# HKUST-KnowComp/DualMessagePassing

Measured on AMD Instinct MI355X. Metric: (pattern,graph) pairs/sec DMPNN fwd+bwd hid=128, higher is better.
Workload: dtype f32

## Files before the change

dualmessagepassing_amd/_abi.py:

```python
import ctypes

c_int = ctypes.c_int
c_i32 = ctypes.c_int32
c_i64 = ctypes.c_int64
c_u64 = ctypes.c_uint64
c_f32 = ctypes.c_float
c_double = ctypes.c_double
c_ptr = ctypes.c_void_p
c_size = ctypes.c_size_t

ABI_VERSION = 97

DMP_COLLATE_MAX_JOBS = 4
DMP_POOL_MAX_JOBS = 4
DMP_REDUCE_MAX_SEGMENTS = 16
DMP_ADAMW_MAX_SKIP = 16
DMP_ADAMW_MAX_SEGMENTS = 1024
DMP_LOOKUP_MAX_JOBS = 8
DMP_CONCAT_MAX_JOBS = 12
DMP_GEMM_MAX_JOBS = 12
DMP_GEMM_MAX_TERMS = 3
DMP_ATB_MAX_JOBS = 8
DMP_MEM_MEAN, DMP_MEM_SUM, DMP_MEM_MAX = 0, 1, 2
DMP_LRP_MAX_NEIGHBOURS = 32
# ... 259 lines not shown
                                   c_ptr, c_ptr, c_int, c_ptr]),
    "dmp_adamw_step_segments": (c_int, [c_ptr, c_ptr, c_ptr, c_ptr, c_ptr, c_i64, c_ptr, c_ptr, c_int, c_ptr, c_ptr, c_ptr, c_double, c_double,
                                        c_double, c_double, c_ptr, c_int, c_ptr]),
    "dmp_adamw_step_guarded": (c_int, [c_ptr, c_ptr, c_ptr, c_ptr, c_ptr, c_i64, c_ptr, c_double, c_double, c_double, c_double,
                                       c_ptr, c_ptr, c_int, c_ptr, c_int, c_ptr]),
    "dmp_edge_select_build": (c_int, [c_ptr, c_ptr, c_ptr, c_ptr, c_i64, c_ptr, c_ptr, c_ptr, c_ptr]),
    "dmp_edge_select_nodes": (c_int, [c_ptr, c_ptr, c_ptr, c_ptr, c_i64, c_ptr, c_ptr, c_ptr, c_ptr]),
    "dmp_edge_fwd_fused": (c_int, [c_ptr, c_i64, c_ptr, c_i64, c_ptr, c_i64, c_i64, c_ptr, c_ptr, c_ptr, c_ptr,
                                   c_i64, c_int, c_f32, c_ptr, c_i64, c_ptr]),
    "dmp_edge_fwd_typed": (c_int, [c_ptr, c_i64, c_ptr, c_i64, c_ptr, c_i64, c_i64, c_ptr, c_ptr, c_ptr, c_ptr, c_ptr,
                                   c_ptr, c_i64, c_i64, c_int, c_f32, c_ptr, c_i64, c_ptr]),
    "dmp_bwd_z_typed_arow": (c_int, [c_ptr, c_i64, c_ptr, c_i64, c_ptr, c_i64, c_i64, c_ptr, c_i64, c_ptr, c_ptr, c_f32,
                                     c_f32, c_ptr, c_ptr, c_ptr, c_ptr, c_i64, c_i64, c_int, c_int, c_ptr, c_i64, c_ptr, c_i64, c_ptr]),
    "dmp_mask_slots": (c_int, [c_ptr, c_i64, c_ptr, c_i64, c_ptr, c_ptr]),
    "dmp_pool_relu_bwd_blocks": (c_i64, [c_i64, c_int]),
    "dmp_pool_relu_bwd": (c_int, [c_ptr, c_i64, c_ptr, c_i64, c_ptr, c_ptr, c_ptr, c_ptr, c_i64, c_i64, c_int, c_f32, c_ptr, c_i64,
                                  c_ptr, c_ptr, c_ptr]),
    "dmp_relu_bwd_gathered_colsum": (c_int, [c_ptr, c_i64, c_ptr, c_ptr, c_ptr, c_i64, c_i64, c_int, c_f32, c_ptr, c_i64, c_ptr, c_ptr]),
    "dmp_dev_set_exact_fp32": (None, [c_int]),
    "dmp_dev_get_exact_fp32": (c_int, []),
    "dmp_rel_gemm": (c_int, [c_ptr, c_i64, c_i64, c_ptr, c_i64, c_int, c_int, c_ptr, c_ptr, c_ptr, c_ptr, c_i64, c_ptr, c_i64,
                             c_int, c_ptr, c_i64, c_ptr]),
    "dmp_rel_atb_blocks": (c_i64, [c_int]),
    "dmp_rel_atb": (c_int, [c_ptr, c_i64, c_i64, c_ptr, c_i64, c_i64, c_ptr, c_ptr, c_ptr, c_ptr, c_int, c_i64, c_int, c_ptr, c_ptr]),
    "dmp_atb_typed_blocks_h": (c_i64, [c_i64, c_int]),
    "dmp_atb_rows_blocks_h": (c_i64, [c_i64, c_int, c_int, c_int]),
    "dmp_atb_rows_plain": (c_int, [c_ptr, c_i64, c_ptr, c_i64, c_ptr, c_i64, c_int, c_int, c_int, c_ptr, c_ptr]),
    "dmp_atb_rows_masked": (c_int, [c_ptr, c_i64, c_ptr, c_i64, c_ptr, c_ptr, c_i64, c_int, c_int, c_int, c_ptr, c_ptr, c_ptr]),
    "dmp_atb_jobs_blocks_h": (c_i64, [c_i64, c_int, c_int]),
    "dmp_atb_rows_jobs_h": (c_int, [_p(dmp_atb_job), c_int, c_i64, c_int, c_ptr, c_ptr, c_ptr, c_i64, c_ptr]),
    "dmp_atb_tile_jobs_blocks": (c_i64, [c_i64, c_int, c_int]),
    "dmp_mfma_partial_rows_h": (c_i64, [c_i64, c_int]),
    "dmp_gemm_k64": (c_int, [c_ptr, c_i64, c_ptr, c_i64, c_int, c_ptr, c_i64, c_i64, c_ptr]),
    "dmp_atb_typed": (c_int, [c_ptr, c_i64, c_ptr, c_i64, c_ptr, c_ptr, c_ptr, c_i64, c_i64, c_int, c_ptr, c_ptr, c_ptr]),
    "dmp_out_fwd_fused_rows": (c_int, [c_ptr, c_i64, c_ptr, c_i64, c_ptr, c_ptr, c_ptr, c_int, c_ptr, c_i64, c_i64, c_int, c_int, c_ptr,
                                       c_i64, c_ptr]),
    "dmp_bwd_h1_fused_rows": (c_int, [c_ptr, c_i64, c_ptr, c_i64, c_ptr, c_i64, c_ptr, c_ptr, c_ptr, c_int, c_i64, c_int, c_f32, c_ptr,
                                      c_i64, c_ptr, c_ptr, c_ptr]),
    "dmp_kept_rows_scratch_words": (c_i64, [c_i64]),
    "dmp_kept_rows": (c_int, [c_ptr, c_i64, c_int, c_ptr, c_ptr, c_ptr, c_ptr]),
    "dmp_l0_edge_fwd_rows": (c_int, [c_ptr, c_i64, c_int, c_ptr, c_i64, c_ptr, c_i64, c_ptr, c_ptr, c_ptr, c_ptr, c_ptr, c_ptr, c_i64, c_int,
                                     c_f32, c_ptr, c_i64, c_ptr]),
    "dmp_l0_bwd_w_rows": (c_int, [c_ptr, c_i64, c_int, c_ptr, c_ptr, c_i64, c_ptr, c_i64, c_ptr, c_ptr, c_i64, c_int, c_ptr, c_ptr]),
    "dmp_typed_partial_rows": (c_i64, [c_i64, c_int]),
    "dmp_out_fwd_typed": (c_int, [_p(dmp_typed_job), c_int, c_ptr, c_ptr, c_ptr, c_i64, c_i64, c_int, c_ptr]),
    "dmp_bwd_h1_typed": (c_int, [c_ptr, c_i64, c_ptr, c_i64, c_ptr, c_i64, c_ptr, c_ptr, c_ptr, c_i64, c_i64, c_int, c_f32, c_ptr, c_i64,
                                 c_ptr, c_ptr, c_ptr]),
    "dmp_kept_rows_jobs": (c_int, [_p(dmp_kept_job), c_int, c_ptr, c_ptr, c_ptr, c_ptr, c_i64, c_ptr, c_ptr, c_ptr, c_ptr]),
    "dmp_row_mask_bits_jobs": (c_int, [_p(dmp_rowmask_job), c_int, c_ptr]),
    "dmp_atb2_blocks": (c_i64, [c_i64, c_int]),
    "dmp_atb2_jobs": (c_int, [_p(dmp_atb2_job), c_int, c_ptr, c_ptr, c_ptr, c_i64, c_i64, c_int, c_ptr]),
    "dmp_bwd_z_w": (c_int, [c_ptr, c_i64, c_ptr, c_i64, c_ptr, c_i64, c_ptr, c_i64, c_i64, c_ptr, c_i64, c_ptr, c_ptr, c_f32, c_f32,
                            c_ptr, c_ptr, c_ptr, c_i64, c_i64, c_int, c_ptr, c_i64, c_ptr, c_i64, c_ptr, c_ptr]),
    "dmp_out_fwd_typed_codes": (c_int, [_p(dmp_typed_job), c_ptr, c_i64, c_int, c_ptr, c_i64, c_i64, c_i64, c_ptr, c_ptr, c_ptr, c_i64, c_i64, c_int, c_ptr]),
    "dmp_bwd_h1_w_blocks": (c_i64, [c_i64]),
    "dmp_bwd_h1_w": (c_int, [c_ptr, c_i64, c_ptr, c_i64, c_ptr, c_i64, c_ptr, c_ptr, c_i64, c_i64, c_int, c_f32, c_ptr, c_i64,
                             c_ptr, c_ptr, c_ptr, c_ptr]),
    "dmp_bwd_h1_w_max_codes": (c_int, []),
    "dmp_bwd_h1_w_codes": (c_int, [c_ptr, c_i64, c_ptr, c_i64, c_ptr, c_i64, c_ptr, c_ptr, c_i64, c_i64, c_int, c_f32, c_ptr, c_i64,
                                   c_ptr, c_ptr, c_ptr, c_ptr, c_i64, c_int, c_ptr, c_i64, c_i64, c_int, c_ptr, c_ptr]),
    "dmp_node_chain_blocks": (c_i64, [c_i64]),
    "dmp_node_chain_panel_words": (c_i64, []),
    "dmp_node_chain_pack": (c_int, [_p(dmp_chain_panel), c_int, c_ptr, c_ptr]),
    "dmp_node_chain_fwd": (c_int, [c_ptr, c_i64, c_ptr, c_i64, c_ptr, c_ptr, c_ptr, c_int, c_f32, c_ptr, c_ptr, c_i64, c_i64, c_int,
                                   c_ptr, c_i64, c_ptr, c_i64, c_ptr, c_i64, c_ptr]),
    "dmp_node_chain_bwd": (c_int, [c_ptr, c_i64, c_ptr, c_i64, c_ptr, c_i64, c_ptr, c_int, c_f32, c_ptr, c_ptr, c_i64, c_i64, c_int,
                                   c_ptr, c_i64, c_ptr, c_i64, c_ptr, c_i64, c_ptr, c_ptr, c_ptr]),
    "dmp_edge_mlp_fwd": (c_int, [c_ptr, c_i64, c_ptr, c_i64, c_ptr, c_i64, c_i64, c_ptr, c_ptr, c_ptr, c_ptr, c_i64, c_int, c_ptr, c_ptr, c_i64,
                                 c_ptr, c_ptr, c_ptr, c_i64, c_i64, c_int, c_f32, c_ptr, c_i64, c_ptr, c_i64, c_ptr]),
    "dmp_l0_edge_mlp_max_codes": (c_int, []),
    "dmp_l0_edge_mlp_fwd": (c_int, [c_ptr, c_i64, c_int, c_ptr, c_i64, c_int, c_i64, c_ptr, c_i64, c_i64, c_ptr, c_ptr, c_ptr, c_ptr, c_f32,
                                    c_ptr, c_i64, c_int, c_ptr, c_ptr, c_i64, c_i64, c_ptr, c_i64, c_i64, c_ptr, c_ptr, c_i64, c_i64, c_int,
                                    c_ptr, c_i64, c_ptr, c_i64, c_ptr]),
    "dmp_row_mask_bits": (c_int, [c_ptr, c_i64, c_ptr, c_ptr]),
    "dmp_row_mask_rows": (c_int, [c_ptr, c_i64, c_int, c_i64, c_ptr, c_ptr]),
    "dmp_bwd_z_fused": (c_int, [c_ptr, c_i64, c_ptr, c_i64, c_ptr, c_i64, c_i64, c_ptr, c_i64, c_ptr, c_ptr, c_ptr,
                                c_f32, c_f32, c_i64, c_int, c_ptr, c_i64, c_ptr]),
    "dmp_gemm_k128": (c_int, [c_ptr, c_i64, c_ptr, c_i64, c_int, c_ptr, c_i64, c_i64, c_int, c_ptr]),
    "dmp_edge_combine": (c_int, [c_ptr, c_i64, c_ptr, c_i64, c_ptr, c_ptr, c_ptr, c_ptr, c_ptr, c_i64,
                                 c_int, c_int, c_f32, c_ptr, c_i64, c_ptr]),
    "dmp_relu_bwd_g_colsum": (c_int, [c_ptr, c_i64, c_ptr, c_i64, c_ptr, c_ptr, c_i64, c_int, c_f32, c_ptr, c_i64,
                                      c_ptr, c_ptr]),
    "dmp_edge_combine_bwd_g": (c_int, [c_ptr, c_i64, c_ptr, c_ptr, c_i64, c_int, c_ptr, c_i64, c_ptr]),
    "dmp_compgcn_agg": (c_int, [c_ptr, c_i64, c_ptr, c_i64, c_ptr, c_ptr, c_ptr, c_ptr, c_i64, c_int, c_int,
                                c_ptr, c_i64, c_ptr]),
    "dmp_compgcn_agg_bwd": (c_int, [c_ptr, c_i64, c_ptr, c_i64, c_ptr, c_i64, c_ptr, c_ptr, c_ptr, c_ptr,
                                    c_i64, c_int, c_int, c_ptr, c_i64, c_ptr, c_i64, c_ptr]),
    "dmp_attn_supported_dh": (c_int, [c_int]),
    "dmp_attn_fwd": (c_int, [c_ptr, c_ptr, c_ptr, c_ptr, c_ptr, c_i64, c_i64, c_i64, c_int, c_int, c_f32, c_ptr, c_ptr, c_ptr, c_ptr]),
    "dmp_attn_bwd": (c_int, [c_ptr, c_ptr, c_ptr, c_ptr, c_ptr, c_ptr, c_ptr, c_ptr, c_i64, c_i64, c_i64, c_int, c_int, c_f32, c_ptr,
                             c_ptr, c_ptr, c_ptr, c_ptr]),
    "dmp_mem_init_fwd": (c_int, [c_ptr, c_i64, c_ptr, c_i64, c_ptr, c_i64, c_i64, c_int, c_int, c_int, c_int, c_int, c_ptr, c_ptr,
                                 c_ptr, c_ptr, c_ptr, c_ptr, c_ptr]),
    "dmp_mem_init_bwd": (c_int, [c_ptr, c_ptr, c_ptr, c_ptr, c_ptr, c_i64, c_i64, c_int, c_int, c_int, c_int, c_ptr, c_ptr, c_ptr]),
    "dmp_cnn_fwd": (c_int, [c_ptr, c_i64, c_i64, c_int, c_ptr, c_ptr, c_int, c_int, c_int, c_int, c_int, c_f32, c_ptr, c_int, c_ptr,
                            c_ptr, c_ptr, c_ptr, c_ptr]),
    "dmp_cnn_route_bwd": (c_int, [c_ptr, c_ptr, c_ptr, c_i64, c_i64, c_i64, c_int, c_int, c_int, c_f32, c_ptr, c_ptr]),
    "dmp_cnn_wgrad_chunks": (c_i64, [c_i64]),
    "dmp_cnn_wgrad": (c_int, [c_ptr, c_ptr, c_i64, c_i64, c_i64, c_int, c_int, c_int, c_ptr, c_ptr]),
    "dmp_rnn_fwd": (c_int, [c_ptr, c_ptr, c_ptr, c_ptr, c_ptr, c_i64, c_i64, c_int, c_int, c_int, c_ptr, c_ptr, c_ptr, c_ptr]),
    "dmp_rnn_bwd": (c_int, [c_ptr, c_ptr, c_ptr, c_ptr, c_ptr, c_i64, c_i64, c_int, c_int, c_int, c_ptr, c_ptr]),
    "dmp_relconv_supported": (c_int, [c_int, c_int]),
    "dmp_relconv_fwd": (c_int, [c_ptr, c_ptr, c_ptr, c_ptr, c_ptr, c_ptr, c_ptr, c_i64, c_int, c_int, c_int, c_int, c_int, c_ptr,
                                c_ptr]),
    "dmp_relconv_bwd": (c_int, [c_ptr, c_ptr, c_ptr, c_ptr, c_ptr, c_ptr, c_ptr, c_i64, c_int, c_int, c_int, c_int, c_int, c_ptr,
                                c_ptr]),
# ... 29 lines not shown
```

dualmessagepassing_amd/csrc/dmp_agg.hip:

```cpp
#include "dmp_common.h"

namespace dmp {

static thread_local char g_last_err[256] = "";
void set_last_hip_error(hipError_t e) {
  const char *s = hipGetErrorString(e);
  int i = 0;
  for (; s && s[i] && i < 255; ++i) g_last_err[i] = s[i];
  g_last_err[i] = 0;
}

namespace {

__device__ __forceinline__ float4 ld4(const float *p) {
  return *reinterpret_cast<const float4 *>(p);
}
__device__ __forceinline__ void st4(float *p, const float4 &v) {
  *reinterpret_cast<float4 *>(p) = v;
}
__device__ __forceinline__ float4 zero4() { return make_float4(0.f, 0.f, 0.f, 0.f); }
__device__ __forceinline__ void add4(float4 &a, const float4 &b) {
  a.x += b.x; a.y += b.y; a.z += b.z; a.w += b.w;
}
__device__ __forceinline__ float4 mul4(const float4 &a, float s) {
// ... 32 lines not shown
  if (rowlist) {
    if (row >= *rowcount) return;
    row = rowlist[row];
    if (!ptr_by_pos) prow = row;
  }
  const int beg = rowptr[prow], end = rowptr[prow + 1];
  for (int c0 = 0; c0 < H; c0 += G * 4) {
    const int c = c0 + lane * 4;
    const bool act = c < H;
    float4 a0 = zero4(), a1 = zero4();
    for (int base = beg; base < end; base += G) {
      const int cnt = min(G, end - base);
      int my = 0;
      float myw = 1.f;
      if (lane < cnt) {
        my = ent[base + lane];
        if (WEIGHTED) myw = ew[my >> 1];
      }
      for (int j = 0; j < cnt; j += U) {
        float4 v[U];
        int e[U];
#pragma unroll
        for (int k = 0; k < U; ++k) {
          e[k] = __shfl(my, min(j + k, G - 1), G);
          float w = 1.f;
          if (WEIGHTED) w = __shfl(myw, min(j + k, G - 1), G);
          if (act && j + k < cnt) {
            if (WEIGHTED && w == 0.f) {
              v[k] = zero4();
            } else {
              v[k] = ld4(M + (int64_t)(e[k] >> 1) * ldm + c);
              if (WEIGHTED) v[k] = mul4(v[k], w);
            }
          }
        }
#pragma unroll
        for (int k = 0; k < U; ++k) {
          if (act && j + k < cnt) {
            if (SPLIT && (e[k] & 1)) add4(a1, v[k]); else add4(a0, v[k]);
          }
        }
      }
    }
    if (act) {
      float *o = out + (int64_t)row * ldo + c;
      if (SPLIT) {
        st4(o, mul4(a0, s0));
        st4(o + H, mul4(a1, s1));
      } else {
        st4(o, a0);
      }
    }
  }
}

constexpr int kTileRows = 512, kTileCols = 32, kTilePad = 36, kTileThreads = 512;
struct TileSpec { const int64_t *node_off, *edge_off; int64_t Ba, Bb; int ka, kb; };

__global__ __launch_bounds__(kTileThreads, 2) void seg_sum_tiled(
    const float *__restrict__ M, int64_t ldm, const int32_t *__restrict__ rowptr, const int32_t *__restrict__ ent,
    const TileSpec ts, int H, float s0, float s1, float *__restrict__ out, int64_t ldo, int nslice) {
  __shared__ float rows[kTileRows * kTilePad];
  constexpr int kPieces = kTileRows * 8 / kTileThreads, kRowStep = kTileThreads / 8;
  const int64_t tile = blockIdx.x / nslice;
  const int c0 = (int)(blockIdx.x % nslice) * kTileCols;
  const int64_t tiles_a = ts.Ba > 0 ? (ts.Ba + ts.ka - 1) / ts.ka : 0;
  int64_t g0, g1;
  if (tile < tiles_a) { g0 = tile * ts.ka; g1 = g0 + ts.ka < ts.Ba ? g0 + ts.ka : ts.Ba; }
  else { g0 = ts.Ba + (tile - tiles_a) * ts.kb; g1 = g0 + ts.kb < ts.Ba + ts.Bb ? g0 + ts.kb : ts.Ba + ts.Bb; }
  const int64_t n0 = ts.node_off[g0], n1 = ts.node_off[g1], e0 = ts.edge_off[g0];
  const int R = (int)(ts.edge_off[g1] - e0);
  const int q = threadIdx.x & 7, r0 = threadIdx.x >> 3;
  float4 v[kPieces];
  {
    const float *src = M + (e0 + r0) * ldm + c0 + q * 4;
#pragma unroll
    for (int k = 0; k < kPieces; ++k)
      if (r0 + k * kRowStep < R) v[k] = ld4(src + (int64_t)k * kRowStep * ldm);
  }
  const int64_t row0 = n0 + r0;
  int beg0 = 0, end0 = 0, my0 = 0, my1 = 0;
  if (row0 < n1) {
    beg0 = rowptr[row0]; end0 = rowptr[row0 + 1];
    if (beg0 + q < end0) my0 = ent[beg0 + q];
    if (beg0 + 8 + q < end0) my1 = ent[beg0 + 8 + q];
  }
#pragma unroll
  for (int k = 0; k < kPieces; ++k)
    if (r0 + k * kRowStep < R) *reinterpret_cast<float4 *>(&rows[(r0 + k * kRowStep) * kTilePad + q * 4]) = v[k];
  __syncthreads();
  auto add_entry = [&](int e, float4 &a0, float4 &a1) {
    const float4 x = *reinterpret_cast<const float4 *>(&rows[((e >> 1) - (int)e0) * kTilePad + q * 4]);
    if (e & 1) add4(a1, x); else add4(a0, x);
  };
  for (int64_t row = row0; row < n1; row += kRowStep) {
    float4 a0 = zero4(), a1 = zero4();
    int beg, end;
    if (row == row0) {
      beg = beg0; end = end0;
      const int c1 = min(8, end - beg), c2 = min(8, end - beg - 8);
#pragma unroll
      for (int j = 0; j < 8; ++j)
        if (j < c1) add_entry(__shfl(my0, j, 8), a0, a1);
#pragma unroll
      for (int j = 0; j < 8; ++j)
        if (j < c2) add_entry(__shfl(my1, j, 8), a0, a1);
// ... 433 lines not shown
                        float *out, int64_t ldo, int rows_shared, void *stream,
                        const int32_t *rowlist = nullptr, const int32_t *rowcount = nullptr, int ptr_by_pos = 0) {
  if (N < 0 || H <= 0 || ldm < H || ldo < (split ? 2 * H : H)) return DMP_ERR_BAD_ARG;
  if (N == 0) return DMP_OK;
  if (!rowptr || !out) return DMP_ERR_BAD_ARG;
  if (rowlist && (!rowcount || !M || !ent || !vec_ok(H, {ldm, ldo}, {M, out}) || rows_shared == 3 || (rows_shared == 2 && !split) || ew)) return DMP_ERR_UNSUPPORTED;
  if (N >= kMaxRows) return DMP_ERR_UNSUPPORTED;
  hipStream_t st = (hipStream_t)stream;
  if (!M || !ent) {
    const size_t width = sizeof(float) * (size_t)(split ? 2 * H : H);
    hipError_t e = hipMemset2DAsync(out, sizeof(float) * (size_t)ldo, 0, width, (size_t)N, st);
    if (e != hipSuccess) { set_last_hip_error(e); return DMP_ERR_HIP; }
    return DMP_OK;
  }
  if (vec_ok(H, {ldm, ldo}, {M, out})) {
    DMP_DISPATCH_G(H, {
      const unsigned nb = blocks_for(N, kBlock / G);
      if (rows_shared) {
        if (split) { if (ew) DMP_SS(true, true, true); else if (rows_shared == 2) DMP_SS_INC(); else if (rows_shared == 3) DMP_SS_TAG2(); else DMP_SS(true, false, true); }
        else { if (ew) DMP_SS(false, true, true); else DMP_SS(false, false, true); }
      } else {
        if (split) { if (ew) DMP_SS(true, true, false); else DMP_SS(true, false, false); }
        else { if (ew) DMP_SS(false, true, false); else DMP_SS(false, false, false); }
      }
    });
  } else {
    const unsigned nb = blocks_for(N, kBlock / kWave);
    if (split) seg_sum_scalar<true><<<nb, kBlock, 0, st>>>(M, ldm, rowptr, ent, ew, (int)N, H, s0, s1, out, ldo);
    else seg_sum_scalar<false><<<nb, kBlock, 0, st>>>(M, ldm, rowptr, ent, ew, (int)N, H, s0, s1, out, ldo);
  }
  return check_launch();
}

int dmp_seg_sum(const float *M, int64_t ldm, const int32_t *rowptr, const int32_t *ent,
                const float *edge_w, int64_t num_nodes, int H, float *out, int64_t ldo,
                int rows_shared, void *stream) {
  return seg_sum_impl(M, ldm, rowptr, ent, edge_w, num_nodes, H, false, 1.f, 1.f, out, ldo, rows_shared, stream);
}

int dmp_seg_sum2(const float *M, int64_t ldm, const int32_t *rowptr, const int32_t *ent,
                 const float *edge_w, int64_t num_nodes, int H, float s0, float s1, float *out,
                 int64_t ldo, int rows_shared, void *stream) {
  return seg_sum_impl(M, ldm, rowptr, ent, edge_w, num_nodes, H, true, s0, s1, out, ldo, rows_shared, stream);
}

int dmp_seg_sum2_rows(const float *M, int64_t ldm, const int32_t *rowptr, const int32_t *ent, const int32_t *rowlist,
                      const int32_t *rowcount, int ptr_by_pos, int incidence, int64_t num_nodes, int H, float s0, float s1, float *out,
                      int64_t ldo, void *stream) {
  if (!rowlist || !rowcount) return DMP_ERR_BAD_ARG;
  return seg_sum_impl(M, ldm, rowptr, ent, nullptr, num_nodes, H, true, s0, s1, out, ldo, incidence ? 2 : 1, stream, rowlist, rowcount,
                      ptr_by_pos ? 1 : 0);
}

int dmp_seg_sum2_tiled(const float *M, int64_t ldm, const int32_t *rowptr, const int32_t *ent, const int64_t *node_off,
                       const int64_t *edge_off, int64_t Ba, int64_t Bb, int ka, int kb, int H, float s0, float s1,
                       float *out, int64_t ldo, void *stream) {
  if (Ba < 0 || Bb < 0 || H <= 0 || ldm < H || ldo < 2 * H || (Ba > 0 && ka < 1) || (Bb > 0 && kb < 1)) return DMP_ERR_BAD_ARG;
  if (Ba + Bb == 0) return DMP_OK;
  if (!M || !rowptr || !ent || !node_off || !edge_off || !out) return DMP_ERR_BAD_ARG;
  if (H % kTileCols || ldm % 4 || ldo % 4 || !aligned16(M) || !aligned16(out)) return DMP_ERR_UNSUPPORTED;
  const int64_t tiles = (Ba > 0 ? (Ba + ka - 1) / ka : 0) + (Bb > 0 ? (Bb + kb - 1) / kb : 0);
  TileSpec ts{node_off, edge_off, Ba, Bb, ka > 0 ? ka : 1, kb > 0 ? kb : 1};
  const int nslice = H / kTileCols;
  if (tiles * nslice >= ((int64_t)1 << 31)) return DMP_ERR_UNSUPPORTED;
  seg_sum_tiled<<<(unsigned)(tiles * nslice), kTileThreads, 0, (hipStream_t)stream>>>(M, ldm, rowptr, ent, ts, H, s0, s1, out, ldo, nslice);
  return check_launch();
}

int dmp_gather_rows(const float *X, int64_t ldx, const int32_t *idx, const float *edge_w,
                    int64_t E, int H, float *out, int64_t ldo, void *stream) {
  if (E < 0 || H <= 0 || ldx < H || ldo < H) return DMP_ERR_BAD_ARG;
  if (E == 0) return DMP_OK;
  if (!X || !idx || !out) return DMP_ERR_BAD_ARG;
  if (E >= kMaxRows) return DMP_ERR_UNSUPPORTED;
  hipStream_t st = (hipStream_t)stream;
  if (vec_ok(H, {ldx, ldo}, {X, out})) {
    DMP_DISPATCH_G(H, {
      const unsigned nb = blocks_for(E, (kBlock / G) * 4);
      if (edge_w) gather_rows_vec<G, 4, true><<<nb, kBlock, 0, st>>>(X, ldx, idx, edge_w, E, H, out, ldo);
      else gather_rows_vec<G, 4, false><<<nb, kBlock, 0, st>>>(X, ldx, idx, edge_w, E, H, out, ldo);
    });
  } else {
    gather_rows_scalar<<<blocks_for(E, kBlock / kWave), kBlock, 0, st>>>(X, ldx, idx, edge_w, E, H, out, ldo);
  }
  return check_launch();
}

int dmp_gather_select(const float *D, int64_t ldd, const int32_t *dst, const uint8_t *flag,
                      const float *edge_w, const float *base, int64_t ldb, int64_t E, int H,
                      float s0, float s1, float *out, int64_t ldo, void *stream) {
  if (E < 0 || H <= 0 || ldd < 2 * H || ldo < H || (base && ldb < H)) return DMP_ERR_BAD_ARG;
  if (E == 0) return DMP_OK;
  if (!D || !dst || !out) return DMP_ERR_BAD_ARG;
  if (E >= kMaxRows) return DMP_ERR_UNSUPPORTED;
  hipStream_t st = (hipStream_t)stream;
  if (vec_ok(H, {ldd, ldo, base ? ldb : 0}, {D, out, base})) {
    DMP_DISPATCH_G(H, {
      const unsigned nb = blocks_for(E, (kBlock / G) * 4);
      if (edge_w) gather_select_vec<G, 4, true><<<nb, kBlock, 0, st>>>(D, ldd, dst, flag, edge_w, base, ldb, E, H, s0, s1, out, ldo);
      else gather_select_vec<G, 4, false><<<nb, kBlock, 0, st>>>(D, ldd, dst, flag, edge_w, base, ldb, E, H, s0, s1, out, ldo);
    });
  } else {
    gather_select_scalar<<<blocks_for(E, kBlock / kWave), kBlock, 0, st>>>(D, ldd, dst, flag, edge_w, base, ldb, E, H, s0, s1, out, ldo);
  }
  return check_launch();
}
// ... 99 lines not shown
```

dualmessagepassing_amd/csrc/dmp_common.h:

```cpp
#pragma once
#include <hip/hip_runtime.h>
#include <stdint.h>

#include "../../include/dmp_hip.h"

namespace dmp {

constexpr int kWave = 64;
constexpr int kBlock = 256;
constexpr int kXcds = 8;

__device__ __forceinline__ int xcd_remap(int orig, int nwg) {
  const int q = nwg / kXcds, r = nwg % kXcds, xcd = orig % kXcds;
  const int base = xcd < r ? xcd * (q + 1) : r * (q + 1) + (xcd - r) * q;
  return base + orig / kXcds;
}

void set_last_hip_error(hipError_t e);

inline int check_launch() {
  hipError_t e = hipGetLastError();
  if (e != hipSuccess) {
    set_last_hip_error(e);
    return DMP_ERR_HIP;
  }
  return DMP_OK;
}

constexpr int kMaxDevices = 64;
inline bool opt_in_lds(const void *kernel, int bytes, bool (&done)[kMaxDevices]) {
  int dev = 0;
  if (hipGetDevice(&dev) != hipSuccess || dev < 0 || dev >= kMaxDevices) dev = 0;
  if (done[dev]) return true;
  const hipError_t e = hipFuncSetAttribute(kernel, hipFuncAttributeMaxDynamicSharedMemorySize, bytes);
  if (e != hipSuccess) { set_last_hip_error(e); return false; }
  done[dev] = true;
  return true;
}

inline unsigned one_per_cu_blocks(int64_t tiles_bound) {
  const int64_t cap = 256;
  return (unsigned)(tiles_bound < cap ? (tiles_bound > 0 ? tiles_bound : 1) : cap);
}

inline bool aligned16(const void *p) { return (reinterpret_cast<uintptr_t>(p) & 15u) == 0; }

inline bool slope_ok(float a) { return a >= 0.f && a <= 1.f; }
__device__ __forceinline__ float act_fwd(float x, float a) { return fmaxf(x, a * x); }
__device__ __forceinline__ float act_bwd(float y, float d, float a) { return y > 0.f ? d : a * d; }

}
```

dualmessagepassing_amd/csrc/dmp_fused.hip:

```cpp
#include <math.h>

#include "dmp_common.h"

namespace dmp {
namespace {

constexpr int kMaxPartials = 1024;
constexpr int kU = 4;

__device__ __forceinline__ float4 ld4(const float *p) { return *reinterpret_cast<const float4 *>(p); }
__device__ __forceinline__ void st4(float *p, const float4 &v) { *reinterpret_cast<float4 *>(p) = v; }
__device__ __forceinline__ float4 zero4() { return make_float4(0.f, 0.f, 0.f, 0.f); }
__device__ __forceinline__ void add4(float4 &a, const float4 &b) { a.x += b.x; a.y += b.y; a.z += b.z; a.w += b.w; }
__device__ __forceinline__ float4 mul4(const float4 &a, float s) { return make_float4(a.x * s, a.y * s, a.z * s, a.w * s); }

enum { OP_GATE_RES = 0, OP_SCALE_CS = 1, OP_RELU_BWD_CS = 2, OP_BWD_G_CS = 3, OP_COLSUM = 4, OP_RELU_BWD_G_CS = 5,
       OP_ADD_BIAS_RELU = 6, OP_RELU_BWD_GATHER_CS = 7 };

struct RowArgs {
  const float *a; int64_t lda;
  const float *b; int64_t ldb;
  const float *rowscale;
  const int32_t *dst;
  float *out; int64_t ldo;
// ... 465 lines not shown
#pragma unroll
      for (int k = 0; k < K; ++k) {
        const float x = __builtin_bit_cast(float, __builtin_amdgcn_readlane(__builtin_bit_cast(int, mine[u]), k));
#pragma unroll
        for (int c = 0; c < VW; ++c) e.v[c] += x * w[k].v[c];
      }
#pragma unroll
      for (int c = 0; c < VW; ++c) e.v[c] *= g;
      lane_store<VW>(p.out + r * p.ldo + coloff, lane, e);
    }
  }
}

template <int K>
void launch_smallk_fwd(const SmallKFwdArgs &p, int H, int ncols, hipStream_t st) {
  const int64_t chunk = (int64_t)(kBlock / 64) * kSmallRows, nb = (p.R + chunk - 1) / chunk;
  const dim3 grid((unsigned)(nb < 4096 ? nb : 4096), (unsigned)ncols);
  if (H == 128) smallk_embed_k<K, 2><<<grid, kBlock, 0, st>>>(p);
  else smallk_embed_k<K, 1><<<grid, kBlock, 0, st>>>(p);
}

inline unsigned smallk_blocks(int64_t R) {
  const int64_t chunk = (int64_t)(kBlock / 64) * kSmallRows, nb = (R + chunk - 1) / chunk;
  return (unsigned)(nb < kMaxPartials ? (nb > 0 ? nb : 1) : kMaxPartials);
}

template <int K>
void launch_smallk(const SmallKArgs &p, int H, hipStream_t st) {
  const dim3 grid(smallk_blocks(p.R), (unsigned)(p.ncols + (p.D2 ? 1 : 0)));
  if (H == 128) smallk_atb_k<K, 2><<<grid, kBlock, 0, st>>>(p);
  else smallk_atb_k<K, 1><<<grid, kBlock, 0, st>>>(p);
}

template <int K>
static void launch_smallk_jobs(const SmallKJobs &js, unsigned nbmax, int n, int H, hipStream_t st) {
  const dim3 grid(nbmax, 1u, (unsigned)n);
  if (H == 128) smallk_atb_jobs_k<K, 2><<<grid, kBlock, 0, st>>>(js);
  else smallk_atb_jobs_k<K, 1><<<grid, kBlock, 0, st>>>(js);
}

inline int group_lanes(int H) { return H <= 64 ? 16 : (H <= 128 ? 32 : 64); }

inline unsigned grid_for(int64_t R, int G) {
  const int64_t chunk = (int64_t)(kBlock / G) * kU;
  const int64_t nb = (R + chunk - 1) / chunk;
  return (unsigned)(nb < kMaxPartials ? (nb > 0 ? nb : 1) : kMaxPartials);
}


struct PoolBwdArgs {
  const float *h1; int64_t ldh; const float *table; int64_t ldt; const int32_t *rowmap; const float *gate;
  const int32_t *vptr, *vent; int64_t V; int H; float slope;
  float *dpre; int64_t ldp; float *qc; float *partial;
};

template <int G>
__global__ __launch_bounds__(kBlock) void pool_relu_bwd_k(PoolBwdArgs p) {
  constexpr int GPB = kBlock / G;
  __shared__ float4 red[kBlock];
  const int grp = threadIdx.x / G, lane = threadIdx.x % G;
  const int c = lane * 4;
  const bool act = c < p.H;
  float4 cs = zero4();
  for (int64_t ch = (int64_t)blockIdx.x * GPB + grp; ch < p.V; ch += (int64_t)gridDim.x * GPB) {
    const int beg = p.vptr[ch], end = p.vptr[ch + 1];
    float4 q0 = zero4(), q1 = zero4();
    for (int base = beg; base < end; base += kU) {
      int ent = 0, mi = -1;
      float gt = 0.f;
      if (lane < kU && base + lane < end) {
        ent = p.vent[base + lane];
        const int r = ent >> 1;
        mi = p.rowmap[r];
        gt = p.gate ? p.gate[r] : 1.f;
      }
      float4 hv[kU], uv[kU];
      int en[kU], tr[kU];
      float sc[kU];
#pragma unroll
      for (int k = 0; k < kU; ++k) { en[k] = __shfl(ent, k, G); tr[k] = __shfl(mi, k, G); sc[k] = __shfl(gt, k, G); }
      if (!act) continue;
#pragma unroll
      for (int k = 0; k < kU; ++k)
        if (base + k < end) {
          const bool live = sc[k] != 0.f;
          hv[k] = live ? ld4(p.h1 + (int64_t)(en[k] >> 1) * p.ldh + c) : zero4();
          uv[k] = (live && tr[k] >= 0) ? ld4(p.table + (int64_t)tr[k] * p.ldt + c) : zero4();
        }
#pragma unroll
      for (int k = 0; k < kU; ++k)
        if (base + k < end) {
          const float4 u = mul4(uv[k], sc[k]);
          const float4 t = make_float4(act_bwd(hv[k].x, u.x, p.slope), act_bwd(hv[k].y, u.y, p.slope),
                                       act_bwd(hv[k].z, u.z, p.slope), act_bwd(hv[k].w, u.w, p.slope));
          st4(p.dpre + (int64_t)(en[k] >> 1) * p.ldp + c, t);
          add4(cs, t);
          const float4 gh = mul4(hv[k], sc[k]);
          if (en[k] & 1) add4(q1, gh); else add4(q0, gh);
        }
    }
    if (act) {
      st4(p.qc + ch * 2 * p.H + c, q0);
      st4(p.qc + ch * 2 * p.H + p.H + c, q1);
    }
  }
  red[threadIdx.x] = cs;
  __syncthreads();
  if (grp == 0 && act) {
    float4 t = red[lane];
#pragma unroll
    for (int g = 1; g < GPB; ++g) add4(t, red[g * G + lane]);
    st4(p.partial + (int64_t)blockIdx.x * p.H + c, t);
  }
}

template <int OP>
int launch_rowop(const RowArgs &p, hipStream_t st) {
  const int g = group_lanes(p.H);
  if (g == 16) rowop_kernel<16, OP><<<grid_for(p.R, 16), kBlock, 0, st>>>(p);
  else if (g == 32) rowop_kernel<32, OP><<<grid_for(p.R, 32), kBlock, 0, st>>>(p);
  else rowop_kernel<64, OP><<<grid_for(p.R, 64), kBlock, 0, st>>>(p);
  return check_launch();
}

inline bool ok16(const void *q) { return !q || aligned16(q); }

}
}

using namespace dmp;

extern "C" {

int64_t dmp_colsum_partial_rows(int64_t rows, int H) {
  if (rows <= 0 || H <= 0) return 1;
  return (int64_t)grid_for(rows, group_lanes(H));
}

#define DMP_ROW_CHECK(cond) \
  if (!(cond)) return DMP_ERR_BAD_ARG

static int vec_shape_ok(int H, int64_t l0, int64_t l1, int64_t l2) {
  return H > 0 && H % 4 == 0 && l0 % 4 == 0 && l1 % 4 == 0 && l2 % 4 == 0;
}

int dmp_gate_residual(const float *prev, int64_t ldp, const float *upd, int64_t ldu, const float *gate,
                      int64_t R, int H, float *out, int64_t ldo, void *stream) {
  DMP_ROW_CHECK(R >= 0 && H > 0);
  if (R == 0) return DMP_OK;
  DMP_ROW_CHECK(upd && out && ldu >= H && ldo >= H && (!prev || ldp >= H));
  if (!vec_shape_ok(H, prev ? ldp : 0, ldu, ldo) || !ok16(prev) || !ok16(upd) || !ok16(out)) return DMP_ERR_UNSUPPORTED;
  RowArgs p{prev, ldp, upd, ldu, gate, nullptr, out, ldo, nullptr, R, H};
  return launch_rowop<OP_GATE_RES>(p, (hipStream_t)stream);
}

int dmp_add_bias_relu(const float *a, int64_t lda, const float *b, int64_t ldb, const float *bias, int64_t R, int H,
                      float slope, float *out, int64_t ldo, void *stream) {
  DMP_ROW_CHECK(R >= 0 && H > 0);
  if (!slope_ok(slope)) return DMP_ERR_UNSUPPORTED;
  if (R == 0) return DMP_OK;
  DMP_ROW_CHECK(a && b && out && lda >= H && ldb >= H && ldo >= H);
  if (!vec_shape_ok(H, lda, ldb, ldo) || !ok16(a) || !ok16(b) || !ok16(out) || !ok16(bias)) return DMP_ERR_UNSUPPORTED;
  RowArgs p{a, lda, b, ldb, bias, nullptr, out, ldo, nullptr, R, H, slope};
  return launch_rowop<OP_ADD_BIAS_RELU>(p, (hipStream_t)stream);
}

int dmp_scale_rows_colsum(const float *dOut, int64_t ldd, const float *gate, int64_t R, int H, float *dUpd,
                          int64_t ldu, float *partial, void *stream) {
  DMP_ROW_CHECK(R >= 0 && H > 0 && partial);
  if (R == 0) return hipMemsetAsync(partial, 0, sizeof(float) * (size_t)H, (hipStream_t)stream) == hipSuccess ? DMP_OK : DMP_ERR_HIP;
  DMP_ROW_CHECK(dOut && ldd >= H && (!dUpd || ldu >= H) && (!gate || dUpd));
  if (!vec_shape_ok(H, ldd, dUpd ? ldu : 0, 0) || !ok16(dOut) || !ok16(dUpd) || !ok16(partial)) return DMP_ERR_UNSUPPORTED;
  RowArgs p{dOut, ldd, nullptr, 0, gate, nullptr, dUpd, ldu, partial, R, H};
  return launch_rowop<OP_SCALE_CS>(p, (hipStream_t)stream);
}

int dmp_relu_bwd_colsum(const float *dH, int64_t ldh, const float *act, int64_t lda, int64_t R, int H, float slope,
                        float *dPre, int64_t ldp, float *partial, void *stream) {
  DMP_ROW_CHECK(R >= 0 && H > 0 && partial);
  if (!slope_ok(slope)) return DMP_ERR_UNSUPPORTED;
  if (R == 0) return hipMemsetAsync(partial, 0, sizeof(float) * (size_t)H, (hipStream_t)stream) == hipSuccess ? DMP_OK : DMP_ERR_HIP;
  DMP_ROW_CHECK(dH && act && dPre && ldh >= H && lda >= H && ldp >= H);
  if (!vec_shape_ok(H, ldh, lda, ldp) || !ok16(dH) || !ok16(act) || !ok16(dPre) || !ok16(partial)) return DMP_ERR_UNSUPPORTED;
  RowArgs p{dH, ldh, act, lda, nullptr, nullptr, dPre, ldp, partial, R, H, slope};
  return launch_rowop<OP_RELU_BWD_CS>(p, (hipStream_t)stream);
}

int dmp_relu_bwd_gathered_colsum(const float *table, int64_t ldt, const int32_t *rowmap, const float *gate, const float *act,
                                 int64_t lda, int64_t R, int H, float slope, float *dPre, int64_t ldp, float *partial, void *stream) {
  DMP_ROW_CHECK(R >= 0 && H > 0 && partial);
  if (!slope_ok(slope)) return DMP_ERR_UNSUPPORTED;
  if (R == 0) return hipMemsetAsync(partial, 0, sizeof(float) * (size_t)H, (hipStream_t)stream) == hipSuccess ? DMP_OK : DMP_ERR_HIP;
  DMP_ROW_CHECK(table && rowmap && act && dPre && ldt >= H && lda >= H && ldp >= H);
  if (!vec_shape_ok(H, ldt, lda, ldp) || !ok16(table) || !ok16(act) || !ok16(dPre) || !ok16(partial)) return DMP_ERR_UNSUPPORTED;
  RowArgs p{table, ldt, act, lda, gate, rowmap, dPre, ldp, partial, R, H, slope};
  return launch_rowop<OP_RELU_BWD_GATHER_CS>(p, (hipStream_t)stream);
}

int64_t dmp_pool_relu_bwd_blocks(int64_t num_chunks, int H) {
  const int g = group_lanes(H);
  const int64_t nb = (num_chunks + kBlock / g - 1) / (kBlock / g);
  return nb < 1 ? 1 : (nb < kMaxPartials ? nb : kMaxPartials);
}

int dmp_pool_relu_bwd(const float *h1, int64_t ldh, const float *table, int64_t ldt, const int32_t *rowmap, const float *gate,
                      const int32_t *vptr, const int32_t *vent, int64_t num_chunks, int64_t R, int H, float slope, float *dPre,
                      int64_t ldp, float *chunk_sums, float *partial, void *stream) {
  DMP_ROW_CHECK(R >= 0 && num_chunks >= 0 && H > 0 && partial);
  if (!slope_ok(slope)) return DMP_ERR_UNSUPPORTED;
  const int64_t nb = dmp_pool_relu_bwd_blocks(num_chunks, H);
  if (R == 0 || num_chunks == 0)
    return hipMemsetAsync(partial, 0, sizeof(float) * (size_t)H * (size_t)nb, (hipStream_t)stream) == hipSuccess ? DMP_OK : DMP_ERR_HIP;
  DMP_ROW_CHECK(h1 && table && rowmap && vptr && vent && dPre && chunk_sums && ldh >= H && ldt >= H && ldp >= H);
  if (!vec_shape_ok(H, ldh, ldt, ldp) || H > 256 || !ok16(h1) || !ok16(table) || !ok16(dPre) || !ok16(chunk_sums) || !ok16(partial))
    return DMP_ERR_UNSUPPORTED;
  PoolBwdArgs p{h1, ldh, table, ldt, rowmap, gate, vptr, vent, num_chunks, H, slope, dPre, ldp, chunk_sums, partial};
  hipStream_t st = (hipStream_t)stream;
  const int g = group_lanes(H);
  if (g == 16) pool_relu_bwd_k<16><<<(unsigned)nb, kBlock, 0, st>>>(p);
  else if (g == 32) pool_relu_bwd_k<32><<<(unsigned)nb, kBlock, 0, st>>>(p);
  else pool_relu_bwd_k<64><<<(unsigned)nb, kBlock, 0, st>>>(p);
  return check_launch();
}

int dmp_edge_combine_bwd_g_colsum(const float *dY, int64_t ldy, const float *coef, const int32_t *dst,
                                  int64_t E, int H, float *dG, int64_t ldg, float *partial, void *stream) {
  DMP_ROW_CHECK(E >= 0 && H > 0 && partial);
  if (E == 0) return hipMemsetAsync(partial, 0, sizeof(float) * (size_t)H, (hipStream_t)stream) == hipSuccess ? DMP_OK : DMP_ERR_HIP;
  DMP_ROW_CHECK(dY && coef && dst && dG && ldy >= H && ldg >= 2 * H);
  if (!vec_shape_ok(H, ldy, ldg, 0) || !ok16(dY) || !ok16(dG) || !ok16(partial)) return DMP_ERR_UNSUPPORTED;
  RowArgs p{dY, ldy, nullptr, 0, coef, dst, dG, ldg, partial, E, H};
  return launch_rowop<OP_BWD_G_CS>(p, (hipStream_t)stream);
}

int dmp_relu_bwd_g_colsum(const float *dH, int64_t ldh, const float *act, int64_t lda, const float *coef,
                          const int32_t *dst, int64_t E, int H, float slope, float *dG, int64_t ldg, float *partial,
                          void *stream) {
  DMP_ROW_CHECK(E >= 0 && H > 0 && partial);
  if (!slope_ok(slope)) return DMP_ERR_UNSUPPORTED;
  if (E == 0) return hipMemsetAsync(partial, 0, sizeof(float) * (size_t)H, (hipStream_t)stream) == hipSuccess ? DMP_OK : DMP_ERR_HIP;
  DMP_ROW_CHECK(dH && act && coef && dst && dG && ldh >= H && lda >= H && ldg >= 2 * H);
  if (!vec_shape_ok(H, ldh, lda, ldg) || !ok16(dH) || !ok16(act) || !ok16(dG) || !ok16(partial)) return DMP_ERR_UNSUPPORTED;
  RowArgs p{dH, ldh, act, lda, coef, dst, dG, ldg, partial, E, H, slope};
  return launch_rowop<OP_RELU_BWD_G_CS>(p, (hipStream_t)stream);
}

int dmp_colsum_partials(const float *A, int64_t lda, int64_t R, int H, float *partial, void *stream) {
  DMP_ROW_CHECK(R >= 0 && H > 0 && partial);
  if (R == 0) return hipMemsetAsync(partial, 0, sizeof(float) * (size_t)H, (hipStream_t)stream) == hipSuccess ? DMP_OK : DMP_ERR_HIP;
  DMP_ROW_CHECK(A && lda >= H);
  if (!vec_shape_ok(H, lda, 0, 0) || !ok16(A) || !ok16(partial)) return DMP_ERR_UNSUPPORTED;
  RowArgs p{A, lda, nullptr, 0, nullptr, nullptr, nullptr, 0, partial, R, H};
  return launch_rowop<OP_COLSUM>(p, (hipStream_t)stream);
}

int64_t dmp_smallk_atb_blocks(int64_t rows) { return (int64_t)smallk_blocks(rows); }

static int dmp_smallk_atb_cols(const float *X, int64_t ldx, int K, const float *D, int64_t ldd, int ncols, const float *D2, int64_t ldd2,
                        const float *gate, int64_t R, int H, float *partial, void *stream) {
  return dmp_smallk_atb_cols_masked(X, ldx, K, D, ldd, ncols, D2, ldd2, gate, nullptr, R, H, partial, stream);
}

static int smallk_atb_cols_impl(const float *X, int64_t ldx, int K, const float *D, int64_t ldd, int ncols, const float *D2,
                                int64_t ldd2, const float *gate, const uint32_t *rowmask, const int32_t *list, const int32_t *count,
                                int64_t R, int H, float *partial, void *stream) {
  DMP_ROW_CHECK(R >= 0 && K > 0 && partial && ncols >= 0 && ncols + (D2 ? 1 : 0) >= 1 && ncols <= 8);
  if ((H != 128 && H != 64) || K > kSmallK) return DMP_ERR_UNSUPPORTED;
  const int nblk = ncols + (D2 ? 1 : 0);
  if (R == 0) return hipMemsetAsync(partial, 0, sizeof(float) * (size_t)nblk * K * H, (hipStream_t)stream) == hipSuccess ? DMP_OK : DMP_ERR_HIP;
  DMP_ROW_CHECK(X && (D || ncols == 0) && ldx >= K && (ncols == 0 || ldd >= (int64_t)ncols * H) && (!D2 || ldd2 >= H));
  if (ldd % 2 || ldd2 % 2 || (reinterpret_cast<uintptr_t>(D) & 7u) || (reinterpret_cast<uintptr_t>(D2) & 7u) || !ok16(partial))
    return DMP_ERR_UNSUPPORTED;
  SmallKArgs p{X, ldx, K, D, ldd, gate, R, partial, ncols, D2, ldd2, rowmask, list, count};
  hipStream_t st = (hipStream_t)stream;
// ... 257 lines not shown
```

dualmessagepassing_amd/csrc/dmp_h1w.hip:

```cpp
#include <type_traits>

#include "dmp_x6_tile.h"

namespace dmp {
namespace {

struct H1WArgs {
  const float *dO; int64_t ldo;
  const float *H1; int64_t ldh;
  const float *W2; int64_t ldw;
  float *dPre; int64_t ldg;
  int64_t E;
  const int32_t *slot_edge;
  const int32_t *num_tiles;
  float slope;
  float *partial;
  float *partialA;
  float *partialW;
};

constexpr int kHW = 128, kThreadsW = 512;
constexpr int kPlaneB = 32 * 256;
constexpr int kBufB = 3 * kPlaneB;
constexpr int kOpB = 2 * kBufB;
// ... 591 lines not shown
  };

  zero_acc();
  float cur = 0.f, sv = 0.f;
  unsigned long long starts = 0;
  start();
  for (int k = 0; k < mine; ++k) {
    if ((k & 63) == 0) {
      const float last = __shfl(sv, 63);
      sv = k + lane < mine ? p.tile_scale[lo + k + lane] : 0.f;
      float up = __shfl_up(sv, 1);
      if (lane == 0) up = k > 0 ? last : sv;
      starts = __ballot(k + lane < mine && __float_as_uint(sv) != __float_as_uint(up));
    }
    if ((starts >> (k & 63)) & 1ull) {
      if (pb) { emit(cur); zero_acc(); }
    }
    cur = __shfl(sv, k & 63);
    if (k & 1) tile_step(k, s0, s1);
    else tile_step(k, s1, s0);
    lds_barrier();
  }
  emit(cur);
}

inline unsigned atb2_blocks(int64_t tiles_bound, int num_jobs) {
  int64_t g = 256 / (num_jobs > 0 ? num_jobs : 1);
  if (g < 1) g = 1;
  if (g > tiles_bound) g = tiles_bound > 0 ? tiles_bound : 1;
  return (unsigned)g;
}

inline bool atb2_lds_ready() {
  static bool done[kMaxDevices] = {};
  return opt_in_lds(reinterpret_cast<const void *>(&atb2_k), kAtb2LdsBytes, done);
}


struct DzwArgs {
  const float *dPre; int64_t ldp;
  const float *Z; int64_t ldz;
  const float *W; int64_t ldw;
  float *dZ; int64_t ldo;
  int64_t E;
  const int32_t *slot_edge;
  const float *tile_scale;
  const int32_t *num_tiles;
  const int32_t *dst; const uint8_t *flag;
  const float *D; int64_t ldd; int64_t num_nodes;
  const float *base; int64_t ldb;
  const int32_t *rmap; int64_t rowsR;
  float s0, s1;
  float *partialW; int64_t pstride;
};

__global__ __launch_bounds__(kThreadsW, 1) void dzw_k(const DzwArgs p) {
  extern __shared__ __attribute__((aligned(256))) unsigned char lds[];
  float *const scr_all = reinterpret_cast<float *>(lds + kImgB);
  uint32_t *const rowA = reinterpret_cast<uint32_t *>(lds + kImgB + kScrB);
  uint32_t *const rowB = rowA + 3 * kSub, *const rowC = rowB + 3 * kSub, *const rowR = rowC + 3 * kSub;
  const int wave = __builtin_amdgcn_readfirstlane((int)(threadIdx.x >> 6));
  const bool cols = wave >= 4;
  const int lane = threadIdx.x & 63, li = lane & 31, h = lane >> 5;
  const int u = threadIdx.x & 255;
  const int srow = u >> 5, scol = u & 31;
  constexpr uint32_t kNone = 0xFFFFFFFFu, kOOB = 0xFFFFF000u;

  const int ntiles = __builtin_amdgcn_readfirstlane(*p.num_tiles);
  const int chunk = (ntiles + (int)gridDim.x - 1) / (int)gridDim.x;
  const int lo = (int)blockIdx.x * chunk;
  const int hi = lo + chunk < ntiles ? lo + chunk : ntiles;
  const int mine = hi > lo ? hi - lo : 0;
  const rsrc_t rs_slot = make_rsrc(p.slot_edge, (uint32_t)ntiles * (kSub * 4u));
  const srsrc_t rs_X = cols ? make_srsrc(p.Z, p.ldz, p.E) : make_srsrc(p.dPre, p.ldp, p.E);
  const uint32_t op_off = cols ? (uint32_t)kOpB : 0u;
  const uint32_t rows4 = (uint32_t)(p.E * 4);
  const rsrc_t rs_dst = make_rsrc(p.dst, rows4);
  const rsrc_t rs_flag = make_rsrc(p.flag, p.flag ? (uint32_t)p.E : 0u);
  const rsrc_t rs_rmap = make_rsrc(p.rmap, p.rmap ? rows4 : 0u);
  float *const pw_ = p.partialW + (int64_t)blockIdx.x * p.pstride;

  if (mine == 0) {
    float4 *pw4 = reinterpret_cast<float4 *>(pw_);
    for (int m = threadIdx.x; m < kHW * 2 * kHW / 4; m += kThreadsW) pw4[m] = make_float4(0.f, 0.f, 0.f, 0.f);
    return;
  }

  int id_rows[kSubLoads];
  int id_own = -1, own_staged = -1;
  float4 pre[kSubLoads];
  uint32_t pre_a = 0, pre_b = 0;
  int pre_r = -1;
  auto load_ids = [&](int k) {
    const bool ok = k < mine;
    const uint32_t so = (uint32_t)(lo + k) * (kSub * 4u);
#pragma unroll
    for (int m = 0; m < kSubLoads; ++m)
      id_rows[m] = ok ? (int)__builtin_amdgcn_raw_buffer_load_b32(rs_slot, (srow + 8 * m) * 4, (int)so, 0) : -1;
    if (!cols && u < kSub) id_own = ok ? (int)__builtin_amdgcn_raw_buffer_load_b32(rs_slot, u * 4, (int)so, 0) : -1;
  };
  auto load_row = [&](int m) { pre[m] = sbuf_load4(rs_X, id_rows[m], (uint32_t)scol * 16u); };
  auto load_row_scalars = [&]() {
    if (!cols && u < kSub) {
      const uint32_t eo = id_own >= 0 ? (uint32_t)id_own * 4u : kOOB;
      pre_a = __builtin_amdgcn_raw_buffer_load_b32(rs_dst, (int)eo, 0, 0);
      pre_b = __builtin_amdgcn_raw_buffer_load_b8(rs_flag, id_own >= 0 ? id_own : (int)kOOB, 0, 0);
      pre_r = p.rmap ? (id_own >= 0 ? (int)__builtin_amdgcn_raw_buffer_load_b32(rs_rmap, (int)eo, 0, 0) : -1) : id_own;
      own_staged = id_own;
    }
  };
  auto stage_row = [&](int buf, int m) {
    uint2 ph, pm, pl;
    split_pair(pre[m].x, pre[m].y, ph.x, pm.x, pl.x);
    split_pair(pre[m].z, pre[m].w, ph.y, pm.y, pl.y);
    const uint32_t r = (uint32_t)(srow + 8 * m);
    const uint32_t off = op_off + (uint32_t)buf * kBufB + 256u * r + 16u * ((uint32_t)(scol >> 1) ^ swz(r)) + 8u * (uint32_t)(scol & 1);
    *reinterpret_cast<uint2 *>(lds + off) = ph;
    *reinterpret_cast<uint2 *>(lds + off + kPlaneB) = pm;
    *reinterpret_cast<uint2 *>(lds + off + 2 * kPlaneB) = pl;
  };
  auto stage_scalars = [&](int par) {
    if (!cols && u < kSub) {
      const bool ok = own_staged >= 0;
      rowA[par * kSub + u] = ok ? pre_a : kNone;
      rowB[par * kSub + u] = pre_b;
      rowC[par * kSub + u] = ok ? (uint32_t)own_staged : kNone;
      rowR[par * kSub + u] = (ok && p.base && pre_r >= 0) ? (uint32_t)pre_r : kNone;
    }
  };
  float sv = 0.f;
  unsigned long long starts = 0;
  auto class_chunk = [&](int k) {
    const float last = __shfl(sv, 63);
    sv = k + lane < mine ? p.tile_scale[lo + k + lane] : 0.f;
    float up = __shfl_up(sv, 1);
    if (lane == 0) up = k > 0 ? last : sv;
    starts = __ballot(k + lane < mine && __float_as_uint(sv) != __float_as_uint(up));
  };

  load_ids(0);
#pragma unroll
  for (int m = 0; m < kSubLoads; ++m) load_row(m);
  load_row_scalars();
  load_ids(1);

  if (cols) {
    const int pw = wave & 1, qw = (wave >> 1) & 1;
    const int G16 = lane >> 4, q4 = (lane & 15) >> 2, pp = lane & 3;
    auto tr_base = [&](int half) {
      const uint32_t row0 = (uint32_t)(8 * (G16 >> 1) + q4);
      const uint32_t ch0 = (uint32_t)(8 * half + 2 * (G16 & 1) + (pp >> 1));
      const uint32_t sw0 = ((uint32_t)q4 << 2) | (uint32_t)(2 * (G16 >> 1));
      return 256u * row0 + 16u * (ch0 ^ sw0) + 8u * (uint32_t)(pp & 1);
    };
    const uint32_t tA = (uint32_t)kOpB + tr_base(pw), tB = tr_base(qw);
    auto tr_frag = [&](uint32_t base, int buf, int plane, int blk, int kg, Frag8 &f) {
      const uint32_t o0 = (base ^ (uint32_t)(64 * blk)) + (uint32_t)(buf * kBufB + plane * kPlaneB + 4096 * kg);
      const uint32_t o1 = (base ^ (uint32_t)(64 * blk) ^ 16u) + (uint32_t)(buf * kBufB + plane * kPlaneB + 4096 * kg + 1024);
      const v4s x = __builtin_amdgcn_ds_read_tr16_b64_v4i16((lds_v4s_ptr)(lds + o0));
      const v4s y = __builtin_amdgcn_ds_read_tr16_b64_v4i16((lds_v4s_ptr)(lds + o1));
      f.v = __builtin_shufflevector(x, y, 0, 1, 2, 3, 4, 5, 6, 7);
    };
    auto tr_split = [&](uint32_t base, int buf, int blk, int kg, Split8 &sp) {
      tr_frag(base, buf, 0, blk, kg, sp.hi);
      tr_frag(base, buf, 1, blk, kg, sp.mid);
      tr_frag(base, buf, 2, blk, kg, sp.lo);
    };
    f32x16 wacc[2][2];
    auto zero_acc = [&]() {
#pragma unroll
      for (int i = 0; i < 2; ++i)
#pragma unroll
        for (int j = 0; j < 2; ++j)
#pragma unroll
          for (int r = 0; r < 16; ++r) wacc[i][j][r] = 0.f;
    };
    const rsrc_t rs_pw = make_rsrc(pw_, (uint32_t)(kHW * 2 * kHW * 4));
    const uint32_t e_voff = (uint32_t)((64 * pw + 4 * h) * (2 * kHW) + 64 * qw + li) * 4u;
    bool emitted = false;
    auto emit = [&](float c) {
#pragma unroll
      for (int i = 0; i < 2; ++i) {
        float t0[2][16], b0[2][16];
#pragma unroll
        for (int j = 0; j < 2; ++j)
#pragma unroll
          for (int r = 0; r < 16; ++r) {
            const int so = ((32 * i + (r & 3) + 8 * (r >> 2)) * (2 * kHW) + 32 * j) * 4;
            t0[j][r] = emitted ? __uint_as_float(__builtin_amdgcn_raw_buffer_load_b32(rs_pw, (int)e_voff, so, 0)) : 0.f;
            b0[j][r] = emitted ? __uint_as_float(__builtin_amdgcn_raw_buffer_load_b32(rs_pw, (int)e_voff, so + kHW * 4, 0)) : 0.f;
          }
#pragma unroll
        for (int j = 0; j < 2; ++j)
#pragma unroll
          for (int r = 0; r < 16; ++r) {
// ... 54 lines not shown
  const int cs = wave & 3;
  const int col = 32 * cs + li;
  float *const scr = scr_all + cs * (32 * kScrStride);
  const int lrow = lane >> 3, c4 = 32 * cs + (lane & 7) * 4;
  const uint32_t col4 = (uint32_t)c4 * 4u;
  constexpr uint32_t kRowBytes = kHW * 4u;
  const srsrc_t rs_C = make_srsrc(p.dZ, p.ldo, p.E);
  const srsrc_t rs_T = make_srsrc(p.D, p.ldd, p.num_nodes);
  const srsrc_t rs_R = make_srsrc(p.base, p.base ? p.ldb : (int64_t)kHW, p.base ? (p.rmap ? p.rowsR : p.E) : 0);
  constexpr int kGroups = 8;
  Split8 B6[kGroups];
  const rsrc_t rs_W = make_rsrc(p.W, (uint32_t)(kHW * p.ldw * 4));
  const uint32_t w_first = (uint32_t)((int64_t)64 * h * p.ldw + col) * 4u;
  const uint32_t w_step = __builtin_amdgcn_readfirstlane((int)(p.ldw * 4));
  auto load_panel = [&](float c) {
    uint32_t off;
    asm volatile("v_mov_b32 %0, %1" : "=v"(off) : "v"(w_first));
#pragma unroll
    for (int s0 = 0; s0 < 64; s0 += 8) {
      float w0[8], w1[8];
#pragma unroll
      for (int j = 0; j < 8; ++j) {
        w0[j] = __uint_as_float(__builtin_amdgcn_raw_buffer_load_b32(rs_W, (int)off, (int)((s0 + j) * w_step), 0));
        w1[j] = __uint_as_float(__builtin_amdgcn_raw_buffer_load_b32(rs_W, (int)off + (int)kRowBytes, (int)((s0 + j) * w_step), 0));
      }
      float w[8];
#pragma unroll
      for (int j = 0; j < 8; ++j) w[j] = w0[j] + c * w1[j];
      split8(make_float4(w[0], w[1], w[2], w[3]), make_float4(w[4], w[5], w[6], w[7]), B6[s0 / 8]);
      __builtin_amdgcn_sched_barrier(0);
    }
  };
  const uint32_t a0 = 256u * (uint32_t)li + 16u * ((uint32_t)(8 * h) ^ swz((uint32_t)li));
  f32x16 acc;
  float4 g0[4], g1[4];
  auto fetch_operand = [&](int par, int k) {
    const int rr = 8 * k + lrow;
    g0[k] = sbuf_load4(rs_T, (int)rowA[par * kSub + rr], col4 + (rowB[par * kSub + rr] ? kRowBytes : 0u));
    g1[k] = sbuf_load4(rs_R, (int)rowR[par * kSub + rr], col4);
  };
  auto rows_step = [&](int k, int par3) {
    const int buf = k & 1, nxt3 = par3 == 2 ? 0 : par3 + 1;
#pragma unroll
    for (int r = 0; r < 16; ++r) acc[r] = 0.f;
    const unsigned char *img = lds + (uint32_t)buf * kBufB;
    Frag8 ah, am, al;
    ah.v = *reinterpret_cast<const bf16x8 *>(img + a0);
    am.v = *reinterpret_cast<const bf16x8 *>(img + kPlaneB + a0);
    al.v = *reinterpret_cast<const bf16x8 *>(img + 2 * kPlaneB + a0);
    auto action = [&](int i) {
      if (i < 4) {}
      else if (i < 8) stage_row(buf ^ 1, i - 4);
      else if (i == 8) stage_scalars(nxt3);
      else if (i < 13) load_row(i - 9);
      else if (i == 13) load_row_scalars();
      else if (i == 14) load_ids(k + 3);
    };
#pragma unroll
    for (int g = 0; g < kGroups; ++g) {
      Frag8 nh = ah, nm = am, nl = al;
      if (g + 1 < kGroups) {
        const uint32_t an = a0 ^ (uint32_t)(16 * (g + 1));
        nh.v = *reinterpret_cast<const bf16x8 *>(img + an);
        nm.v = *reinterpret_cast<const bf16x8 *>(img + kPlaneB + an);
        nl.v = *reinterpret_cast<const bf16x8 *>(img + 2 * kPlaneB + an);
      }
      const Split8 &bb = B6[g];
      __builtin_amdgcn_sched_barrier(0);
      acc = __builtin_amdgcn_mfma_f32_32x32x16_bf16(al.v, bb.hi.v, acc, 0, 0, 0);
      acc = __builtin_amdgcn_mfma_f32_32x32x16_bf16(ah.v, bb.lo.v, acc, 0, 0, 0);
      acc = __builtin_amdgcn_mfma_f32_32x32x16_bf16(am.v, bb.mid.v, acc, 0, 0, 0);
      __builtin_amdgcn_sched_barrier(0);
      action(2 * g);
      __builtin_amdgcn_sched_barrier(0);
      acc = __builtin_amdgcn_mfma_f32_32x32x16_bf16(am.v, bb.hi.v, acc, 0, 0, 0);
      acc = __builtin_amdgcn_mfma_f32_32x32x16_bf16(ah.v, bb.mid.v, acc, 0, 0, 0);
      acc = __builtin_amdgcn_mfma_f32_32x32x16_bf16(ah.v, bb.hi.v, acc, 0, 0, 0);
      __builtin_amdgcn_sched_barrier(0);
      action(2 * g + 1);
      ah = nh; am = nm; al = nl;
    }
  };
  auto rows_epilogue = [&](int par) {
#pragma unroll
    for (int r = 0; r < 16; ++r) scr[((r & 3) + 8 * (r >> 2) + 4 * h) * kScrStride + li] = acc[r];
    const int nxt = par == 2 ? 0 : par + 1;
#pragma unroll
    for (int k = 0; k < 4; ++k) {
      const int rr = 8 * k + lrow;
      float4 v = *reinterpret_cast<const float4 *>(&scr[rr * kScrStride + (lane & 7) * 4]);
      const float sg = rowB[par * kSub + rr] ? p.s1 : p.s0;
      v.x += g1[k].x + sg * g0[k].x; v.y += g1[k].y + sg * g0[k].y;
      v.z += g1[k].z + sg * g0[k].z; v.w += g1[k].w + sg * g0[k].w;
      sbuf_store4(v, rs_C, (int)rowC[par * kSub + rr], col4);
      fetch_operand(nxt, k);
    }
  };
#pragma unroll
  for (int m = 0; m < kSubLoads; ++m) stage_row(0, m);
  stage_scalars(0);
#pragma unroll
  for (int m = 0; m < kSubLoads; ++m) load_row(m);
  load_row_scalars();
  load_ids(2);
  lds_barrier();
#pragma unroll
  for (int c = 0; c < 4; ++c) fetch_operand(0, c);
  int par3 = 0;
  float c_have = 0.f;
  bool have_panel = false;
  for (int k = 0; k < mine; ++k) {
    if ((k & 63) == 0) class_chunk(k);
    const float c = __shfl(sv, k & 63);
    if (!have_panel || __float_as_uint(c) != __float_as_uint(c_have)) {
      load_panel(c);
      c_have = c;
      have_panel = true;
    }
    rows_step(k, par3);
    lds_barrier();
    rows_epilogue(par3);
    par3 = par3 == 2 ? 0 : par3 + 1;
  }
}

constexpr int kDzwLdsBytes = kImgB + kScrB + 4 * 3 * kSub * 4;
inline bool dzw_lds_ready() {
  static bool done[kMaxDevices] = {};
  return opt_in_lds(reinterpret_cast<const void *>(&dzw_k), kDzwLdsBytes, done);
}

inline unsigned h1w_blocks(int64_t tiles_bound) { return one_per_cu_blocks(tiles_bound); }

template <int MODE>
inline bool h1w_lds_ready() {
  static bool done[kMaxDevices] = {};
  return opt_in_lds(reinterpret_cast<const void *>(&h1w_k<MODE>), MODE == 0 ? kH1WLdsBytes : kH1WCodesLdsBytes, done);
}

inline int h1w_check(const float *dO, int64_t ldo, const float *W2, int64_t ldw, const float *H1, int64_t ldh, const int32_t *slot_edge,
                     const int32_t *num_tiles, int64_t tiles_bound, int64_t E, int H, float *dPre, int64_t ldg) {
  if (!dO || !W2 || !H1 || !dPre || !slot_edge || !num_tiles || ldo < H || ldw < H || ldh < H || ldg < H) return DMP_ERR_BAD_ARG;
  if (ldo % 4 || ldh % 4 || ldg % 4 || !aligned16(dO) || !aligned16(H1) || !aligned16(dPre)) return DMP_ERR_UNSUPPORTED;
  if (!stride_ok(ldo) || !stride_ok(ldh) || !stride_ok(ldg) || E >= ((int64_t)1 << 30) || tiles_bound * kSub * 4 >= ((int64_t)1 << 32) - 8192 ||
      (int64_t)H * ldw * 4 >= ((int64_t)1 << 32) - 8192 || !fits4g(E, ldo) || !fits4g(E, ldh) || !fits4g(E, ldg))
    return DMP_ERR_UNSUPPORTED;
  return DMP_OK;
}

}
}

using namespace dmp;

extern "C" {

int64_t dmp_bwd_h1_w_blocks(int64_t tiles_bound) { return (int64_t)h1w_blocks(tiles_bound); }

int dmp_bwd_h1_w(const float *dO, int64_t ldo, const float *W2, int64_t ldw, const float *H1, int64_t ldh,
                 const int32_t *slot_edge, const int32_t *num_tiles, int64_t tiles_bound, int64_t E, int H, float slope,
                 float *dPre, int64_t ldg, float *partial, float *partial_rows, float *partial_w, void *stream) {
  if (H != 128 || g_exact_fp32) return DMP_ERR_UNSUPPORTED;
  if (E < 0 || tiles_bound < 0) return DMP_ERR_BAD_ARG;
  if (!partial || !partial_w || !aligned16(partial) || !aligned16(partial_w) || (partial_rows && !aligned16(partial_rows))) return DMP_ERR_BAD_ARG;
  if (!slope_ok(slope)) return DMP_ERR_UNSUPPORTED;
  hipStream_t st = (hipStream_t)stream;
  if (E == 0) {
    const size_t rows = (size_t)h1w_blocks(tiles_bound);
    if (hipMemsetAsync(partial, 0, sizeof(float) * H * rows, st) != hipSuccess) return DMP_ERR_HIP;
    if (partial_rows && hipMemsetAsync(partial_rows, 0, sizeof(float) * H * rows, st) != hipSuccess) return DMP_ERR_HIP;
    if (hipMemsetAsync(partial_w, 0, sizeof(float) * H * H * rows, st) != hipSuccess) return DMP_ERR_HIP;
    return DMP_OK;
  }
  if (const int rc = h1w_check(dO, ldo, W2, ldw, H1, ldh, slot_edge, num_tiles, tiles_bound, E, H, dPre, ldg)) return rc;
  if (!h1w_lds_ready<0>()) return DMP_ERR_HIP;
  H1WArgs a{};
  a.dO = dO; a.ldo = ldo; a.H1 = H1; a.ldh = ldh; a.W2 = W2; a.ldw = ldw; a.dPre = dPre; a.ldg = ldg; a.E = E;
  a.slot_edge = slot_edge; a.num_tiles = num_tiles; a.slope = slope; a.partial = partial; a.partialA = partial_rows; a.partialW = partial_w;
  h1w_k<0><<<h1w_blocks(tiles_bound), kThreadsW, kH1WLdsBytes, st>>>(a);
  return check_launch();
}

// ... 9 lines not shown
  if (!partial || !partial_w || !partial_x || !aligned16(partial) || !aligned16(partial_w) || (partial_rows && !aligned16(partial_rows)))
    return DMP_ERR_BAD_ARG;
  if (!slope_ok(slope)) return DMP_ERR_UNSUPPORTED;
  hipStream_t st = (hipStream_t)stream;
  const int nb = residual ? 3 : 2;
  if (E == 0) {
    const size_t rows = (size_t)h1w_blocks(tiles_bound);
    if (hipMemsetAsync(partial, 0, sizeof(float) * H * rows, st) != hipSuccess) return DMP_ERR_HIP;
    if (partial_rows && hipMemsetAsync(partial_rows, 0, sizeof(float) * H * rows, st) != hipSuccess) return DMP_ERR_HIP;
    if (hipMemsetAsync(partial_w, 0, sizeof(float) * H * H * rows, st) != hipSuccess) return DMP_ERR_HIP;
    if (hipMemsetAsync(partial_x, 0, sizeof(float) * K * nb * H * rows, st) != hipSuccess) return DMP_ERR_HIP;
    return DMP_OK;
  }
  if (const int rc = h1w_check(dO, ldo, W2, ldw, H1, ldh, slot_edge, num_tiles, tiles_bound, E, H, dPre, ldg)) return rc;
  if (r1 > r0 && (!enc || !coef_e)) return DMP_ERR_BAD_ARG;
  if (!fits4g(r1 - r0, lde)) return DMP_ERR_UNSUPPORTED;
  H1WCodeArgs a{};
  a.dO = dO; a.ldo = ldo; a.H1 = H1; a.ldh = ldh; a.W2 = W2; a.ldw = ldw; a.dPre = dPre; a.ldg = ldg; a.E = E;
  a.slot_edge = slot_edge; a.num_tiles = num_tiles; a.slope = slope; a.partial = partial; a.partialA = partial_rows; a.partialW = partial_w;
  const int64_t n = r1 - r0;
  a.enc = n > 0 ? enc + r0 * lde : nullptr; a.lde4 = (uint32_t)(lde * 4); a.coef = n > 0 ? coef_e + r0 : nullptr;
  a.enc_bytes = n > 0 ? (uint32_t)(((n - 1) * lde + K) * 4) : 0u;
  a.r0 = (int)r0; a.nrange = (int)n; a.K = K; a.partialX = partial_x;
  if (residual) {
    if (!h1w_lds_ready<2>()) return DMP_ERR_HIP;
    h1w_k<2><<<h1w_blocks(tiles_bound), kThreadsW, kH1WCodesLdsBytes, st>>>(a);
  } else {
    if (!h1w_lds_ready<1>()) return DMP_ERR_HIP;
    h1w_k<1><<<h1w_blocks(tiles_bound), kThreadsW, kH1WCodesLdsBytes, st>>>(a);
  }
  return check_launch();
}


int dmp_bwd_z_w(const float *dPre, int64_t ldp, const float *Z, int64_t ldz, const float *W, int64_t ldw, const float *D, int64_t ldd,
                int64_t num_nodes, const float *base, int64_t ldb, const int32_t *dst, const uint8_t *flag, float s0, float s1,
                const int32_t *slot_edge, const float *tile_scale, const int32_t *num_tiles, int64_t tiles_bound, int64_t E, int H,
                const int32_t *base_map, int64_t base_rows, float *dZ, int64_t ldo, float *partial_w, void *stream) {
  if (H != 128 || g_exact_fp32) return DMP_ERR_UNSUPPORTED;
  if (E < 0 || num_nodes < 0 || tiles_bound < 0 || !partial_w || !aligned16(partial_w)) return DMP_ERR_BAD_ARG;
  hipStream_t st = (hipStream_t)stream;
  if (E == 0) return hipMemsetAsync(partial_w, 0, sizeof(float) * H * 2 * H * (size_t)h1w_blocks(tiles_bound), st) == hipSuccess ? DMP_OK : DMP_ERR_HIP;
  if (!dPre || !Z || !W || !D || !dst || !slot_edge || !tile_scale || !num_tiles || !dZ || ldp < H || ldz < H || ldw < 2 * H || ldd < 2 * H ||
      ldo < H || (base && ldb < H))
    return DMP_ERR_BAD_ARG;
  if (base_map && (!base || base_rows < 0)) return DMP_ERR_BAD_ARG;
  if (ldp % 4 || ldz % 4 || ldo % 4 || ldd % 4 || (base && ldb % 4) || !aligned16(dPre) || !aligned16(Z) || !aligned16(dZ) || !aligned16(D) ||
      (base && !aligned16(base)))
    return DMP_ERR_UNSUPPORTED;
  if (!stride_ok(ldp) || !stride_ok(ldz) || !stride_ok(ldo) || !stride_ok(ldd) || (base && !stride_ok(ldb)) || E >= ((int64_t)1 << 30) ||
      num_nodes >= ((int64_t)1 << 31) || tiles_bound * kSub * 4 >= ((int64_t)1 << 32) - 8192 || (int64_t)H * ldw * 4 >= ((int64_t)1 << 32) - 8192 ||
      !fits4g(E, ldp) || !fits4g(E, ldz) || !fits4g(E, ldo) || (base && !fits4g(base_map ? base_rows : E, ldb)) || !fits4g(num_nodes, ldd))
    return DMP_ERR_UNSUPPORTED;
  if (!dzw_lds_ready()) return DMP_ERR_HIP;
  DzwArgs a{};
  a.dPre = dPre; a.ldp = ldp; a.Z = Z; a.ldz = ldz; a.W = W; a.ldw = ldw; a.dZ = dZ; a.ldo = ldo; a.E = E; a.slot_edge = slot_edge;
  a.tile_scale = tile_scale; a.num_tiles = num_tiles; a.dst = dst; a.flag = flag; a.D = D; a.ldd = ldd; a.num_nodes = num_nodes;
  a.base = base; a.ldb = base ? ldb : H; a.rmap = base_map; a.rowsR = base_rows; a.s0 = s0; a.s1 = s1;
  a.partialW = partial_w; a.pstride = (int64_t)H * 2 * H;
  dzw_k<<<h1w_blocks(tiles_bound), kThreadsW, kDzwLdsBytes, st>>>(a);
  return check_launch();
}

int64_t dmp_atb2_blocks(int64_t tiles_bound, int num_jobs) { return (int64_t)atb2_blocks(tiles_bound, num_jobs); }

int dmp_atb2_jobs(const dmp_atb2_job *jobs, int num_jobs, const int32_t *slot_row, const float *tile_scale, const int32_t *num_tiles,
                  int64_t tiles_bound, int64_t rows, int H, void *stream) {
  if (H != 128 || g_exact_fp32) return DMP_ERR_UNSUPPORTED;
  if (!jobs || num_jobs < 1 || num_jobs > kAtb2MaxJobs || rows < 0 || tiles_bound < 0) return DMP_ERR_BAD_ARG;
  if (!slot_row || !tile_scale || !num_tiles) return DMP_ERR_BAD_ARG;
  if (rows >= ((int64_t)1 << 30) || tiles_bound * kSub * 4 >= ((int64_t)1 << 32) - 8192) return DMP_ERR_UNSUPPORTED;
  Atb2Args a{};
  for (int i = 0; i < num_jobs; ++i) {
    const dmp_atb2_job &j = jobs[i];
    if (!j.partial_T || j.ldp < H || (rows > 0 && (!j.Z || !j.D || j.ldz < H || j.ldd < H))) return DMP_ERR_BAD_ARG;
    if (j.ldz % 4 || j.ldd % 4 || (rows > 0 && (!aligned16(j.Z) || !aligned16(j.D)))) return DMP_ERR_UNSUPPORTED;
    if (!stride_ok(j.ldz) || !stride_ok(j.ldd) || !fits4g(rows, j.ldz) || !fits4g(rows, j.ldd)) return DMP_ERR_UNSUPPORTED;
    a.job[i].Z = j.Z; a.job[i].ldz = j.ldz; a.job[i].D = j.D; a.job[i].ldd = j.ldd; a.job[i].pT = j.partial_T; a.job[i].pB = j.partial_B;
    a.job[i].pstride = j.partial_stride; a.job[i].ldp = j.ldp;
  }
  a.E = rows; a.slot_edge = slot_row; a.tile_scale = tile_scale; a.num_tiles = num_tiles;
  if (!atb2_lds_ready()) return DMP_ERR_HIP;
  atb2_k<<<dim3(atb2_blocks(tiles_bound, num_jobs), (unsigned)num_jobs), kThreadsW, kAtb2LdsBytes, (hipStream_t)stream>>>(a);
  return check_launch();
}

}
```

dualmessagepassing_amd/fused.py:

```python
import ctypes as _ctypes
import os as _os
import threading

import torch
from torch.autograd.function import once_differentiable

from . import _abi, _lib, gatememo, ops, side
from ._lib import check, ptr, stream_ptr


def _partials(rows, H, dev):
    lib = _lib.load()
    return torch.empty((int(lib.dmp_colsum_partial_rows(rows, H)), H), dtype=torch.float32, device=dev)


MAX_REDUCE_SEGMENTS = _abi.DMP_REDUCE_MAX_SEGMENTS


class _Deferred(threading.local):

    def __init__(self):
        self.stack = []


# ... 43 lines not shown
def gate_residual(prev, upd, gate):
    lib = _lib.load()
    R, H = upd.shape
    out = torch.empty_like(upd)
    with _lib.timed("gate_residual[H=%d,R=%d]", (H, R), 4 * H * R * (3 if prev is not None else 2) + (4 * R if gate is not None else 0)):
        check(lib.dmp_gate_residual(ptr(prev), H, ptr(upd), H, ptr(gate), R, H, ptr(out), H, stream_ptr()),
              "dmp_gate_residual")
    return out


def add_bias_relu_(a, b, bias, slope=0.0):
    lib = _lib.load()
    R, H = a.shape
    with _lib.timed("add_bias_relu[H=%d,R=%d]", (H, R), 12 * H * R):
        check(lib.dmp_add_bias_relu(ptr(a), a.stride(0), ptr(b), b.stride(0), ptr(bias), R, H, slope, ptr(a), a.stride(0),
                                    stream_ptr()), "dmp_add_bias_relu")
    return a


def scale_rows_colsum(d_out, gate):
    lib = _lib.load()
    R, H = d_out.shape
    part = _partials(R, H, d_out.device)
    d_upd = torch.empty_like(d_out) if gate is not None else None
    with _lib.timed("scale_rows_colsum[H=%d,R=%d]", (H, R), 4 * H * R * (2 if gate is not None else 1)):
        check(lib.dmp_scale_rows_colsum(ptr(d_out), H, ptr(gate), R, H, ptr(d_upd), H, ptr(part), stream_ptr()),
              "dmp_scale_rows_colsum")
    return (d_upd if gate is not None else d_out), reduce_partials(part)


def relu_bwd_colsum_(d_h, act, out=None, slope=0.0):
    lib = _lib.load()
    R, H = d_h.shape
    part = _partials(R, H, d_h.device)
    dst = d_h if out is None else out
    ldo = dst.stride(0) if R > 1 else H
    with _lib.timed("relu_bwd_colsum[H=%d,R=%d]", (H, R), 12 * H * R):
        check(lib.dmp_relu_bwd_colsum(ptr(d_h), H, ptr(act), H, R, H, slope, ptr(dst), ldo, ptr(part), stream_ptr()),
              "dmp_relu_bwd_colsum")
    return dst, reduce_partials(part)


def relu_bwd_gathered_colsum(table, rowmap, gate, act, slope=0.0):
    lib = _lib.load()
    R, H = act.shape
    part = _partials(R, H, act.device)
    out = torch.empty((R, H), dtype=torch.float32, device=act.device)
    with _lib.timed("relu_bwd_gathered[H=%d,R=%d]", (H, R), 8 * H * R + 8 * R + 4 * H * table.size(0)):
        check(lib.dmp_relu_bwd_gathered_colsum(ptr(table), table.stride(0), ptr(rowmap), ptr(gate), ptr(act), act.stride(0), R, H,
                                               slope, ptr(out), H, ptr(part), stream_ptr()), "dmp_relu_bwd_gathered_colsum")
    return out, reduce_partials(part)


def pool_relu_bwd(table, rowmap, gate, act, pool, slope=0.0, skip_dead=False, chunk_sums=False):
    lib = _lib.load()
    R, H = act.shape
    V = pool.num_chunks
    nb = int(lib.dmp_pool_relu_bwd_blocks(V, H))
    part = torch.empty((nb, H), dtype=torch.float32, device=act.device)
    kc = keep_pool_csr(pool, gate) if skip_dead else None
    vptr, vent = (pool.vptr, pool.vent) if kc is None else kc
    out = dead_rows_buffer((R, H), act.device) if kc is not None else torch.empty((R, H), dtype=torch.float32, device=act.device)
    qc = torch.empty((V, 2 * H), dtype=torch.float32, device=act.device)
    with _lib.timed("pool_relu_bwd[H=%d,R=%d]", (H, R), 8 * H * R + 12 * R + 8 * H * V):
        check(lib.dmp_pool_relu_bwd(ptr(act), act.stride(0), ptr(table), table.stride(0), ptr(rowmap), ptr(gate), ptr(vptr),
                                    ptr(vent), V, R, H, slope, ptr(out), H, ptr(qc), ptr(part), stream_ptr()), "dmp_pool_relu_bwd")
    if chunk_sums:
        return out, reduce_partials(part), qc
    Q = ops.seg_sum_raw(qc, pool.gptr, pool.gent, pool.num_graphs, None, False, rows_shared=False)
    return out, reduce_partials(part), Q


def keep_pool_csr(pool, gate):
    own = None if gate is None else gatememo.owner(gate)
    if not has_row_mask(own, True, True) or pool.num_chunks == 0 or gate.numel() == 0:
        return None
    return gatememo.memo(own, ("keep_pool", id(pool)), (pool,), lambda: _csr_keep(pool.vptr, pool.vent, gate, pool.num_chunks), True)


def _csr_keep_buffers(rows, entries, device):
    nscr = int(_lib.load().dmp_csr_keep_scratch_words(rows))
    ws = torch.empty(nscr + rows + 1 + entries, dtype=torch.int32, device=device)
    return ws[:nscr], ws[nscr:nscr + rows + 1], ws[nscr + rows + 1:]


def _csr_keep(csr_ptr, csr_ent, gate, rows):
    row_cnt, kptr, kent = _csr_keep_buffers(rows, csr_ent.numel(), csr_ptr.device)
    check(_lib.load().dmp_csr_keep(ptr(csr_ptr), ptr(csr_ent), ptr(gate.reshape(-1)), rows, csr_ent.numel(), ptr(row_cnt), ptr(kptr),
                                   ptr(kent), stream_ptr()), "dmp_csr_keep")
    return kptr, kent


def pool_rows(x, pool, weight=None):
    return ops.seg_sum_raw(pool_chunk_sums(x, pool, weight), pool.gptr, pool.gent, pool.num_graphs, None, False, rows_shared=False)


def pool_chunk_sums(x, pool, weight=None):
    split = pool.flag8 is not None
    kc = keep_pool_csr(pool, weight) if (weight is not None and x.size(1) % 4 == 0 and x.is_contiguous()) else None
    if kc is not None:
        return ops.seg_sum_raw(x, kc[0], kc[1], pool.num_chunks, None, split, 1.0, 1.0, rows_shared=False)
    return ops.seg_sum_raw(x, pool.vptr, pool.vent, pool.num_chunks, weight, split, 1.0, 1.0, rows_shared=False)


USE_POOL_ALGEBRA = True
POOL_ALGEBRA_WIDTHS = (64, 128)


def _aligned(*tensors):
    return all(t is None or (t.dtype == torch.float32 and t.is_contiguous() and t.data_ptr() % 16 == 0) for t in tensors)


def pool_algebra_ok(index, H, epool, eW2, eb2):
    return bool(USE_POOL_ALGEBRA and H in POOL_ALGEBRA_WIDTHS and getattr(epool, "rows_in_order", False) and epool.num_graphs > 0
                and index.num_edges > 0 and typed_ok(index, H) and eb2 is not None and _aligned(eW2, eb2))


def pool_out(partH, partZ, pool, gcnt, W2, b2, partX=None, vpool=None, want_q=False):
    lib = _lib.load()
# ... 224 lines not shown
        return hit
    if device.type == "cuda" and torch.cuda.is_current_stream_capturing():
        return None
    bound = (R + 31) // 32
    slot = torch.arange(bound * 32, dtype=torch.int32, device=device)
    slot[R:] = -1
    res = (slot, const_zeros(bound, device), torch.tensor([bound], dtype=torch.int32, device=device), bound)
    if len(_IDENTITY_TILES) < 64:
        _IDENTITY_TILES[key] = res
    return res


def ascending_tiles(gate):
    mask = binary_gate_mask(gate)
    if mask is None:
        return None

    def build():
        R = gate.numel()
        lst, cnt = kept_rows(mask, 0, R, tiles=True)
        bound = (R + 31) // 32
        return lst, const_zeros(bound, mask.device), cnt[1:2], bound

    return gatememo.memo(gate, "ascending_tiles", (), build)


def bwd_z_typed(d_pre, ld_pre, Wes, d_s, base, coef, index, WesT=None, base_map=None, gate=None, dead_rows=None, dst=None):
    lib = _lib.load()
    E, H = d_pre.size(0), Wes.size(0)
    lt = live_tiles(index, coef, gate) if dead_rows is not None else None
    ms = lt[0] if lt is not None else masked_slots(index, coef, gate)
    if ms is None:
        dead_rows = None
    out = (torch.zeros((E, H), dtype=torch.float32, device=d_pre.device) if dead_rows == "zero" else
           dead_rows_buffer((E, H), d_pre.device) if dead_rows == "leave" else torch.empty((E, H), dtype=torch.float32, device=d_pre.device))
    if WesT is None:
        WesT = torch.cat([Wes[:, :H].t(), Wes[:, H:].t()], dim=1)
    d_s = d_s.contiguous()
    if lt is not None:
        slot_edge, tile_scale, num_tiles, bound = lt
    else:
        slot_edge, tile_scale, num_tiles, bound = index.class_tiles(coef)
        if dead_rows is not None:
            slot_edge = ms
    with _lib.timed("bwd_z_typed[H=%d,E=%d]", (H, E), 4 * H * E * (3 if base is not None else 2) + 5 * E):
        check(lib.dmp_bwd_z_typed_arow(ptr(d_pre), ld_pre, ptr(WesT), WesT.size(1), ptr(d_s), d_s.size(1), index.num_nodes,
                                       ptr(base), base.stride(0) if base is not None else H, ptr(index.dst32 if dst is None else dst), ptr(index.rev8), -1.0, 1.0,
                                       ptr(slot_edge), ptr(ms), ptr(tile_scale), ptr(num_tiles), bound, E, H, 1,
                                       ptr(base_map), base.size(0) if base_map is not None else 0, ptr(out), H, stream_ptr()),
              "dmp_bwd_z_typed")
    return out


def bwd_z_w(d_pre, z, Wes, d_s, base, coef, index, WesT=None, base_map=None, gate=None, dead_rows=None, dst=None):
    lib = _lib.load()
    E, H = d_pre.size(0), Wes.size(0)
    lim = (1 << 32) - 65536
    if ((dead_rows is None) != (gate is None) or H != 128 or lib.dmp_dev_get_exact_fp32() or z is None or z.size(0) != E or E * H * 4 >= lim
            or E * d_pre.stride(0) * 4 >= lim or E * z.stride(0) * 4 >= lim or d_pre.data_ptr() % 16 or z.data_ptr() % 16
            or d_pre.stride(0) % 4 or z.stride(0) % 4 or index.num_nodes * d_s.size(1) * 4 >= lim):
        return None
    if gate is None:
        if getattr(index, "_coef_deg", None) is None or index._coef_deg[0] is not coef or index.num_edges == 0:
            return None
        lt = index.class_tiles(coef)
    else:
        lt = live_tiles(index, coef, gate)
    if lt is None:
        return None
    if base is not None and (base.stride(0) % 4 or base.data_ptr() % 16 or base.size(0) * base.stride(0) * 4 >= lim):
        return None
    slot_edge, tile_scale, num_tiles, bound = lt
    out = (torch.zeros((E, H), dtype=torch.float32, device=d_pre.device) if dead_rows == "zero" else
           dead_rows_buffer((E, H), d_pre.device) if dead_rows == "leave" else torch.empty((E, H), dtype=torch.float32, device=d_pre.device))
    if WesT is None:
        WesT = torch.cat([Wes[:, :H].t(), Wes[:, H:].t()], dim=1)
    d_s = d_s.contiguous()
    G = int(lib.dmp_bwd_h1_w_blocks(bound))
    part = torch.empty((G, H * 2 * H), dtype=torch.float32, device=d_pre.device)
    with _lib.timed("bwd_z_w[H=%d,E=%d]", (H, E), 4 * H * E * (4 if base is not None else 3) + 5 * E):
        check(lib.dmp_bwd_z_w(ptr(d_pre), d_pre.stride(0), ptr(z), z.stride(0), ptr(WesT), WesT.size(1), ptr(d_s), d_s.size(1), index.num_nodes,
                              ptr(base), base.stride(0) if base is not None else H, ptr(index.dst32 if dst is None else dst), ptr(index.rev8), -1.0, 1.0,
                              ptr(slot_edge), ptr(tile_scale), ptr(num_tiles), bound, E, H, ptr(base_map),
                              base.size(0) if base_map is not None else 0, ptr(out), H, ptr(part), stream_ptr()), "dmp_bwd_z_w")
    return out, reduce_partials(part).view(H, 2 * H)


USE_ATB2 = True


def atb2_ok(a, b, H):
    lib = _lib.load()
    lim = (1 << 32) - 65536
    return bool(USE_ATB2 and H == 128 and not lib.dmp_dev_get_exact_fp32() and a.size(0) == b.size(0) and a.size(0) * a.stride(0) * 4 < lim
                and b.size(0) * b.stride(0) * 4 < lim and a.stride(0) % 4 == 0 and b.stride(0) % 4 == 0
                and a.data_ptr() % 16 == 0 and b.data_ptr() % 16 == 0)


def atb2(pairs, tiles, wide=False):
    lib = _lib.load()
    slot, tile_scale, num_tiles, bound = tiles
    n, H = len(pairs), 128
    R = pairs[0][0].size(0)
    G = int(lib.dmp_atb2_blocks(bound, n))
    W = 2 * H if wide else H
    jobs = (_abi.dmp_atb2_job * n)()
    parts = []
    for j, (a, b) in enumerate(pairs):
        part = torch.empty((G, H * W), dtype=torch.float32, device=a.device)
        parts.append(part)
        jobs[j].Z, jobs[j].ldz, jobs[j].D, jobs[j].ldd = a.data_ptr(), a.stride(0), b.data_ptr(), b.stride(0)
        jobs[j].partial_T, jobs[j].partial_B = part.data_ptr(), (part.data_ptr() + 4 * H if wide else None)
        jobs[j].partial_stride, jobs[j].ldp = H * W, W
    with _lib.timed("atb2[jobs=%d,R=%d]", (n, R), 8 * H * R * n):
        check(lib.dmp_atb2_jobs(jobs, n, ptr(slot), ptr(tile_scale), ptr(num_tiles), bound, R, H, stream_ptr()), "dmp_atb2_jobs")
    return [reduce_partials(part).view(H, W) for part in parts]


def atb_typed(z, d_pre, coef, index, gate=None, plain=False):
    lib = _lib.load()
    E, H = z.shape
    lt = live_tiles(index, coef, gate)
    if plain and lt is not None:
        at = ascending_tiles(gate)
        if at is not None:
            lt = at
    if lt is not None:
        slot_edge, tile_scale, num_tiles, bound = lt
    else:
        slot_edge, tile_scale, num_tiles, bound = index.class_tiles(coef)
        ms = masked_slots(index, coef, gate)
        if ms is not None:
            slot_edge = ms
    if atb2_ok(z, d_pre, H):
        return atb2([(z, d_pre)], (slot_edge, tile_scale, num_tiles, bound), wide=not plain)[0]
    G = int(lib.dmp_atb_typed_blocks_h(bound, H))
    if plain:
# ... 1284 lines not shown
    Q = pool_rows(H1e, epool, e_gate).view(G_ * halves, H)
    gcnt = pool_weight_sums(epool, e_gate)
    cnt = gcnt.view(G_ * halves, 1)
    zs = pool_rows(z, epool, e_gate if zero_rows_gate(e_gate) else None).view(G_ * halves, H) if c.residual else None
    if Q.is_contiguous() and eW2.is_contiguous() and Q.size(0) <= SMALL_GEMM_MAX_ROWS:
        es = torch.empty((G_ * halves, H), dtype=torch.float32, device=Q.device)
        small_gemm_jobs([(es, [(Q, False, eW2, True), (cnt, False, eb2.view(1, H), False)], zs)])
    else:
        es = torch.addmm(zs, Q, eW2.t()) if c.residual else Q @ eW2.t()
        es.addcmul_(cnt, eb2.view(1, H))
    return vs, es.view(G_, halves * H)[:, :H], gcnt


def _grad_seeds(c, x, z, H1e, dxn, dzn, dvs, des, typed):
    H = c.H
    lazy = None
    if dvs is not None:
        exp = ops.gather_rows_raw(dvs.contiguous(), c.vpool.seg32)
        dxn = exp if dxn is None else dxn + exp
    if des is not None:
        ep = c.epool
        if dzn is None and typed and H1e.size(0) > 0 and des.size(1) == H:
            lazy = (des.contiguous(), pool_rowmap(ep), ep)
        else:
            if ep.flag8 is not None and des.size(1) == H:
                des = torch.cat([des, torch.zeros_like(des)], dim=1)
            exp = (ops.gather_select_raw(des.contiguous(), ep.seg32, ep.flag8, H, None, 1.0, 1.0) if ep.flag8 is not None
                   else ops.gather_rows_raw(des.contiguous(), ep.seg32))
            dzn = exp if dzn is None else dzn + exp
    if dxn is None:
        dxn = torch.zeros_like(x)
    if dzn is None and lazy is None:
        dzn = torch.zeros_like(z)
    return dxn.contiguous(), (dzn.contiguous() if dzn is not None else None), lazy


def l0_tables_full(l0, tables, W0):
    return all(r[1] > r[0] and n[1] > n[0] for _, r, n in tables) and len(tables) * l0.K == W0.size(0)


def l0_codes_buffer(l0, tables, W0, residual, H, device):
    return (torch.empty if l0_tables_full(l0, tables, W0) else torch.zeros)((W0.size(0), (3 if residual else 2) * H),
                                                                           dtype=torch.float32, device=device)


def l0_codes_block(c, tables, device, walked):
    if not h1w_codes_ok(c.l0, tables or (), walked):
        return None
    t, rows, _ = tables[-1]
    XX, K0 = l0_codes_buffer(c.l0, tables, c.W0, c.residual, c.H, device), c.l0.K
    return XX, dict(enc=c.l0.enc, K=K0, coef_e=c.index.edge_select(c.coef)[2], rows=rows, residual=c.residual, out=XX[t * K0:(t + 1) * K0])


def _edge_out_bwd_lazy(c, H1e, lazy, gcnt):
    H, e_gate = c.H, c.e_gate
    T, emap, ep = lazy
    if c.poolalg:
        T = T if _aligned(T) else T.clone(memory_format=torch.contiguous_format)
        skip = c.l0 is None and c.nd is not None and USE_PLAIN_ATB and dead_edge_rows(c.index, H, e_gate, c.coef)
        dG, dbe, qc = pool_relu_bwd(rows_gemm(T, c.eW2, False), emap, e_gate, H1e, ep, c.slope, skip_dead=skip, chunk_sums=True)
        if gcnt is None:
            gcnt = pool_weight_sums(ep, e_gate)
        dW2e, db2e = pool_wgrad(qc, ep, T, gcnt)
        return dG, dbe, dW2e, db2e
    if H % 4 == 0 and H <= 256:
        skip = c.l0 is None and c.nd is not None and USE_PLAIN_ATB and dead_edge_rows(c.index, H, e_gate, c.coef)
        dG, dbe, Q = pool_relu_bwd(T @ c.eW2, emap, e_gate, H1e, ep, c.slope, skip_dead=skip)
        Q = Q[:, :H]
    else:
        dG, dbe = relu_bwd_gathered_colsum(T @ c.eW2, emap, e_gate, H1e, c.slope)
        Q = pool_rows(H1e, ep, e_gate)[:, :H]
    dW2e = T.t() @ Q
    if gcnt is None:
        gcnt = pool_weight_sums(ep, e_gate)
    return dG, dbe, dW2e, gcnt[:, 0] @ T


def _edge_out_bwd_typed(c, tables, H1e, dzn):
    ix, coef, H, slope, e_gate, eW2 = c.index, c.coef, c.H, c.slope, c.e_gate, c.eW2
    l0_XX = None
    if binary_gate_mask(e_gate) is not None:
        skip = USE_MASKED_SUMS and dead_h1_rows(ix, H, e_gate) and (c.l0 is None or c.l0.enc_mask is not None)
        lt = live_tiles(ix, coef, e_gate) if skip else None
        if lt is not None and h1w_ok(dzn, H1e, H):
            l0_XX = l0_codes_block(c, tables, dzn.device, "kept")
            dG, dbe, db2e, dW2e = bwd_h1_w(dzn, eW2, H1e, ascending_tiles(e_gate) or lt, slope, codes=l0_XX and l0_XX[1])[:4]
        elif lt is not None:
            dG, dbe, db2e = bwd_h1_typed(dzn, eW2, H1e, ascending_tiles(e_gate) or lt, slope)
            dW2e = atb_typed(dzn, H1e, coef, ix, gate=e_gate, plain=True)
        else:
            dG, dbe, db2e = bwd_h1_mfma(dzn, eW2, H1e, coef, ix, both_halves=False, gate=e_gate, slope=slope, rows_colsum=True,
                                        skip_dead_stores=skip)
            dW2e = atb_rows(dzn, H1e, e_gate, colsum=False)[0]
        return dG, dbe, dW2e, db2e, l0_XX
    it = identity_tiles(dzn.size(0), dzn.device) if (e_gate is None and h1w_ok(dzn, H1e, H)) else None
    if it is not None:
        l0_XX = l0_codes_block(c, tables, dzn.device, "all")
        dG, dbe, db2e, dW2e = bwd_h1_w(dzn, eW2, H1e, it, slope, codes=l0_XX and l0_XX[1])[:4]
    else:
        dW2e, db2e = atb_rows(dzn, H1e, e_gate)
        dG, dbe = bwd_h1_mfma(dzn, eW2, H1e, coef, ix, both_halves=False, gate=e_gate, slope=slope)
    return dG, dbe, dW2e, db2e, l0_XX


def _edge_out_bwd(c, tables, H1e, dzn, lazy, gcnt, typed):
    if lazy is not None:
        return _edge_out_bwd_lazy(c, H1e, lazy, gcnt) + (None,)
    if typed:
        return _edge_out_bwd_typed(c, tables, H1e, dzn)
    dOe, db2e = scale_rows_colsum(dzn, c.e_gate)
    dW2e = atb(dOe, H1e)
    dH1e = dOe @ c.eW2
    dG, dbe = relu_bwd_g_colsum(dH1e, H1e, c.coef, c.index.dst32, c.slope)
    return dG, dbe, dW2e, db2e, None


def _endpoint_sums(c, dG, typed, device):
    ix, H, N, nd, e_gate = c.index, c.H, c.N, c.nd, c.e_gate
    dXP = dead_rows_buffer((N, 3 * H), device) if nd is not None else torch.empty((N, 3 * H), dtype=torch.float32, device=device)
    sums_masked = typed and USE_MASKED_SUMS and has_row_mask(e_gate)
    if kept_incidence_sums(ix, H, e_gate, nd is not None):
        kp, ke = nd.kept_incidence(ix, e_gate)
        ops.seg_sum_raw(dG[:, :H], kp, ke, N, None, True, 1.0, -1.0, out=dXP[:, H:], rows=nd.rows, ptr_by_pos=True, tag="seg_sum2_kept_inc",
                        incidence=True)
    else:
        nodes = (nd.mask, nd.sel[:2]) if (nd is not None and sums_masked and ops.graph_seg_ok(ix, dG[:, :H], H, dXP[:, H:])) else None
        ops.endpoint_sums(dG[:, :H], ix, out=dXP[:, H:], mask=gate_row_mask(e_gate) if sums_masked else None,
                          gate=e_gate if sums_masked else None, nodes=nodes)
    return dXP


def _l0_edge_code_products(c, tables, dG, dzn, l0_XX):
    l0, e_gate, K0 = c.l0, c.e_gate, c.l0.K
    XX = l0_XX[0] if l0_XX is not None else l0_codes_buffer(l0, tables, c.W0, c.residual, c.H, dG.device)
    for t, rows, _ in (tables[:-1] if l0_XX is not None else tables):
        if rows[1] > rows[0]:
            l0_bwd_w(l0.enc, K0, c.index.edge_select(c.coef)[2], dG, dzn if c.residual else None, rows, XX[t * K0:(t + 1) * K0],
                     mask=(gate_row_mask(e_gate) if (l0.enc_mask is not None and binary_gate_mask(e_gate) is not None)
                           else l0.enc_mask))
    return XX


def _edge_first_wgrad(c, z, dG, typed, want_dz):
    ix, H, e_gate = c.index, c.H, c.e_gate
    if typed and want_dz and H == 128 and (e_gate is None or dead_edge_rows(ix, H, e_gate, c.coef)):
        return None
    return atb_typed(z, dG, c.coef, ix, gate=e_gate) if typed else atb(z, dG)


def _wgrad(a, b, kernel):
    return atb_rows(a, b, colsum=False)[0] if kernel else atb(a, b)


def _node_one_launch(c, x, S, H1n, dxn, dXP):
    one_launch = onepanel_ok(c.H) and atb_ok(dxn, H1n) and atb_ok(x, dXP) and (S is None or atb_ok(S, dXP))
    if c.nd is not None and not (one_launch and binary_gate_mask(c.v_gate) is not None):
        raise _lib.DmpError("fused layer backward: the kept-node path needs the masked weight-gradient launch")
    return one_launch


def _node_out_bwd(c, dxn, H1n, dXP, own_dW2n, kernel):
    nd, H, slope, v_gate, nW2 = c.nd, c.H, c.slope, c.v_gate, c.nW2
    dW2n = db2n = None
    if nd is not None:
        dPn, dbn, db2n = bwd_h1_typed(dxn, nW2, H1n, nd.tiles, slope, out=dXP[:, :H])
        if own_dW2n:
            dW2n = atb_rows(dxn, H1n, v_gate, colsum=False)[0]
    elif onepanel_ok(H) and atb_ok(dxn, H1n):
        if binary_gate_mask(v_gate) is not None:
            dPn, dbn, db2n = bwd_h1_mfma(dxn, nW2, H1n, both_halves=False, gate=v_gate, out=dXP[:, :H], slope=slope,
                                         rows_colsum=True)
            if own_dW2n:
                dW2n = atb_rows(dxn, H1n, v_gate, colsum=False)[0]
        else:
            if own_dW2n:
                dW2n, db2n = atb_rows(dxn, H1n, v_gate)
            dPn, dbn = bwd_h1_mfma(dxn, nW2, H1n, both_halves=False, gate=v_gate, out=dXP[:, :H], slope=slope)
    else:
        dOn, db2n = scale_rows_colsum(dxn, v_gate)
        dW2n = _wgrad(dOn, H1n, kernel)
        dH1n = dOn @ nW2
        dPn, dbn = relu_bwd_colsum_(dH1n, H1n, out=dXP[:, :H], slope=slope)
    return dPn, dbn, db2n, dW2n


def _node_wgrads(c, products):
    nd, v_gate = c.nd, c.v_gate
    last = products[-1] + (None, False)
    if nd is not None:
        res = atb_rows_multi([(a, b, None, False) for a, b in products], tiles=nd.tiles)
        return [r[0] for r in res], None
    vm = binary_gate_mask(v_gate)
    if vm is not None:
        res = atb_rows_multi([(a, b, None, False, vm) for a, b in products[:-1]] + [last])
        return [r[0] for r in res], None
    vm = gate_row_mask(v_gate)
    res = atb_rows_multi([products[0] + (v_gate, True, vm)] + [(a, b, None, False, vm) for a, b in products[1:-1]] + [last])
    return [r[0] for r in res], res[0][1]

# ... 151 lines not shown
            jobs.append((dWx[:, b3 * H:(b3 + 1) * H], [(WV0, True, Yn[b3], False)], None))
        jobs.append((dWV0, [(Yn[b3], False, Wx[:, b3 * H:(b3 + 1) * H], True) for b3 in range(3)], Yn[3] if c.residual else None))
    small_gemm_jobs(jobs)
    return dBn, dWx, dWes, dW0, dWV0


class _FusedDMPLayer(torch.autograd.Function):

    @staticmethod
    def forward(ctx, index, coef, residual, x, z, v_gate, e_gate, Bn, bn, Wx, Wes, be, nW2, nb2, eW2, eb2,
                WesT=None, nW2t=None, eW2t=None, slope=0.0, vpool=None, epool=None, l0=None, W0=None, WV0=None, edge_rows=True,
                inner=0):
        _lib.require_gpu(x, z)
        H = Bn.size(1)
        x, z = x.contiguous(), z.contiguous()
        sums_only = epool is not None and not edge_rows
        c = _LayerCall(index=index, coef=coef, residual=residual, H=H, N=index.num_nodes, slope=slope, inner=int(inner),
                       v_gate=v_gate, e_gate=e_gate, Bn=Bn.contiguous(), bn=bn, Wx=Wx.contiguous(), Wes=Wes.contiguous(), be=be,
                       nW2=nW2, nb2=nb2, eW2=eW2, eb2=eb2, WesT=WesT, nW2t=nW2t, eW2t=eW2t, l0=l0,
                       W0=None if l0 is None else W0.detach(), WV0=None if (l0 is None or WV0 is None) else WV0.detach(),
                       nd=_kept_nodes(index, H, v_gate, l0), vpool=vpool, epool=epool,
                       poolalg=sums_only and pool_algebra_ok(index, H, epool, eW2, eb2))
        S = S0 = M0 = tables = xn = chain_panels = None
        if l0 is not None:
            S0, M0, tables, H1n, P, ldp = _node_first_codes(c, x, z)
        else:
            S, H1n, P, ldp, xn, chain_panels = _node_first_rows(c, x, z)
        if xn is None:
            xn = _node_out(c, x, H1n)
        if l0 is not None:
            H1e, zn = _edge_first_codes(c, z, M0, tables, P, ldp, sums_only)
        else:
            H1e, zn = _edge_first_rows(c, z, P, ldp, sums_only)
        if zn is None and not sums_only:
            zn = _edge_out(c, z, H1e)
        ctx.call, ctx.chain_panels, ctx.l0_S0, ctx.l0_tables, ctx.gcnt = c, chain_panels, S0, tables, None
        ctx.save_for_backward(x, z if l0 is None else None, S, H1n, H1e)
        if vpool is None and epool is None:
            return xn, zn
        ctx.set_materialize_grads(False)
        vs, es, ctx.gcnt = _pooled_outputs(c, z, xn, zn, H1e, sums_only)
        return xn, zn, vs, es

    @staticmethod
    @once_differentiable
    def backward(ctx, dxn, dzn, dvs=None, des=None):
        x, z, S, H1n, H1e = ctx.saved_tensors
        c, tables = ctx.call, ctx.l0_tables
        typed = typed_ok(c.index, c.H)
        want_dx, want_dz = ctx.needs_input_grad[3], ctx.needs_input_grad[4]
        dxn, dzn, lazy = _grad_seeds(c, x, z, H1e, dxn, dzn, dvs, des, typed)
        dz = dW0 = dWV0 = None
        with deferred_reductions():
            dG, dbe, dW2e, db2e, l0_XX = _edge_out_bwd(c, tables, H1e, dzn, lazy, ctx.gcnt, typed)
            dXP = _endpoint_sums(c, dG, typed, x.device)
            if c.l0 is not None:
                XX = _l0_edge_code_products(c, tables, dG, dzn, l0_XX)
                dbn, dWx, dW2n, db2n, Xn, Yn, dx = _node_bwd_codes(c, tables, ctx.l0_S0, x, H1n, dxn, dXP, want_dx)
            else:
                dWes = _edge_first_wgrad(c, z, dG, typed, want_dz)
                dBn, dbn, dWx, dW2n, db2n, dS, dx = _node_bwd_rows(c, ctx.chain_panels, x, S, H1n, dxn, dXP, want_dx)
                if want_dz:
                    dz, dWes = _edge_input_grad(c, z, dG, dS, dzn, lazy, dWes, typed)
        if c.l0 is not None:
            dBn, dWx, dWes, dW0, dWV0 = _l0_final_products(c, XX, Xn, Yn, dWx)
        return (None, None, None, dx, dz, None, None, dBn, dbn, dWx, dWes, dbe, dW2n, db2n, dW2e, db2e, None, None, None, None,
                None, None, None, dW0, dWV0, None, None)


def l0_z_from_codes(index, H, eg, l0, live_edges, residual):
    return bool(USE_OUT_CODES and (live_edges or eg is None) and residual and l0 is not None and H == 128
                and not _lib.load().dmp_dev_get_exact_fp32() and l0.enc.stride(0) % 4 == 0 and l0.enc.data_ptr() % 16 == 0
                and index.num_edges * 128 * 4 < (1 << 32) - 65536)


def l0_dead_inputs(index, H, vg, eg, l0, coef):
    return (l0 is not None and dead_edge_rows(index, H, eg, coef),
            bool(l0 is not None and l0.venc is not None and kept_node_path(index, H, vg, l0)))


def activation_slope(act):
    if type(act) is torch.nn.ReLU:
        return 0.0
    if type(act) is torch.nn.LeakyReLU and 0.0 <= float(act.negative_slope) <= 1.0:
        return float(act.negative_slope)
    return None


def l0_ok(index, H, enc_p, enc_g, W_p, W_g):
    return (USE_LAYER0 and H in MFMA_WIDTHS and enc_p.size(1) == enc_g.size(1) == W_g.size(0) == W_p.size(0) <= L0_KMAX
            and W_g.size(1) == W_p.size(1) == H and W_g.dtype == W_p.dtype == enc_p.dtype == enc_g.dtype == torch.float32
            and enc_p.stride(1) == 1 and enc_g.stride(1) == 1 and enc_g.is_cuda and index.num_edges > 0 and typed_ok(index, H)
            and onepanel_ok(H))


def l0_nodes_ok(H, enc_p, enc_g, W_p, W_g):
    return (enc_p.size(1) == enc_g.size(1) == W_g.size(0) == W_p.size(0) <= SMALLK_MAX and W_g.size(1) == W_p.size(1) == H
            and W_g.dtype == W_p.dtype == enc_p.dtype == enc_g.dtype == torch.float32 and enc_p.stride(1) == 1
            and enc_g.stride(1) == 1 and enc_g.is_cuda and H in MFMA_WIDTHS)


def fused_dmp_layer(index, coef, residual, x, z, v_gate, e_gate, layer, folded=None, pools=None, l0=None, inner=0):
    n2, e2 = layer.nmlp[2], layer.emlp[2]
    Bn, bn, Wx, Wes, be, WesT, nW2t, eW2t = folded if folded is not None else fold_layers([layer])[0]
    vpool, epool = pools[:2] if pools is not None else (None, None)
    edge_rows = pools[2] if pools is not None and len(pools) > 2 else True
    return _FusedDMPLayer.apply(index, coef, bool(residual), x, z, v_gate, e_gate, Bn, bn, Wx, Wes, be,
# ... 3 lines not shown
```

dualmessagepassing_amd/ops.py:

```python
import torch
from torch.autograd.function import once_differentiable

from . import _abi, _lib
from ._lib import check, ptr, stream_ptr


def _mat(t, min_cols=None):
    if t.dtype != torch.float32:
        raise _lib.DmpError("feature matrices must be float32, got %s" % t.dtype)
    if t.dim() != 2:
        raise _lib.DmpError("feature matrices must be 2-D, got shape %s" % (tuple(t.shape),))
    if t.size(0) <= 1:
        t = t.contiguous()
        return t, max(t.size(1), 1)
    if t.stride(1) != 1 or t.stride(0) < t.size(1):
        t = t.contiguous()
    return t, t.stride(0)


def _vec(t, dtype):
    if t is None:
        return None
    if t.dtype != dtype:
        raise _lib.DmpError("expected %s tensor, got %s" % (dtype, t.dtype))
# ... 58 lines not shown
                                                     ka, kb, H, 1.0, -1.0, ptr(out), out.stride(0) if N > 1 else 2 * H, ptr(mask), E,
                                                     None if nodes is None else ptr(nodes[0]), N, stream_ptr()),
                      "dmp_seg_sum2_graphs_masked")
            else:
                check(lib.dmp_seg_sum2_graphs(ptr(M), M.stride(0), ptr(sel_a), ptr(sel_b), ptr(node_off), ptr(edge_off), Ba, Bb, ka, kb,
                                              H, 1.0, -1.0, ptr(out), out.stride(0) if N > 1 else 2 * H, stream_ptr()),
                      "dmp_seg_sum2_graphs")
        return out
    inc_ptr, inc_ent = index.incidence()
    if gate is not None:
        return seg_sum_raw(M, inc_ptr, inc_ent, N, gate.reshape(-1), True, 1.0, -1.0, rows_shared=2, out=out)
    return seg_sum_raw(M, inc_ptr, inc_ent, N, None, True, 1.0, -1.0, rows_shared=2, out=out, tiling=index.tiling)


def seg_sum_raw(M, rowptr, ent, num_nodes, edge_w=None, split=False, s0=1.0, s1=1.0, rows_shared=True, out=None, tiling=None,
                rows=None, ptr_by_pos=False, tag=None, incidence=False):
    lib = _lib.load()
    _lib.require_gpu(M, rowptr, ent, edge_w)
    M, ldm = _mat(M)
    H = M.size(1)
    width = 2 * H if split else H
    if out is None:
        out = torch.empty((num_nodes, width), dtype=torch.float32, device=M.device)
    elif out.shape != (num_nodes, width) or out.dtype != torch.float32 or (num_nodes > 1 and out.stride(1) != 1):
        raise _lib.DmpError("seg_sum: bad out tensor")
    ldo = out.stride(0) if num_nodes > 1 else max(out.size(1), 1)
    ew = _vec(edge_w, torch.float32)
    nent = ent.numel()
    src_rows = min(nent, M.size(0))
    nbytes = 4 * H * src_rows + 4 * out.size(1) * num_nodes + 4 * nent + 4 * (num_nodes + 1) + (4 * nent if ew is not None else 0)
    if split and tiling is not None and USE_TILED_SEG_SUM and ew is None and H % 32 == 0 and ldm % 4 == 0 and ldo % 4 == 0 \
            and M.data_ptr() % 16 == 0 and out.data_ptr() % 16 == 0 and num_nodes > 0:
        node_off, edge_off, Ba, Bb, ka, kb = tiling
        if True:
            with _lib.timed("seg_sum2_tiled[H=%d,rows=%d,ent=%d]", (H, num_nodes, nent), nbytes):
                check(lib.dmp_seg_sum2_tiled(ptr(M), ldm, ptr(rowptr), ptr(ent), ptr(node_off), ptr(edge_off), Ba, Bb, ka, kb, H,
                                             s0, s1, ptr(out), ldo, stream_ptr()), "dmp_seg_sum2_tiled")
            return out
    if rows is not None:
        if not split or ew is not None:
            raise _lib.DmpError("seg_sum: a row list goes with the split sum without weights")
        with _lib.timed((tag or "seg_sum2") + "[H=%d,rows=%d,ent=%d]", (H, num_nodes, nent), nbytes):
            check(lib.dmp_seg_sum2_rows(ptr(M), ldm, ptr(rowptr), ptr(ent), ptr(rows[0]), ptr(rows[1]), int(bool(ptr_by_pos)), int(bool(incidence)),
                                        num_nodes, H, s0, s1, ptr(out), ldo, stream_ptr()), "dmp_seg_sum2_rows")
        return out
    if split:
        with _lib.timed("seg_sum2[H=%d,rows=%d,ent=%d]", (H, num_nodes, nent), nbytes):
            check(lib.dmp_seg_sum2(ptr(M), ldm, ptr(rowptr), ptr(ent), ptr(ew), num_nodes, H, s0, s1,
                                   ptr(out), ldo, int(rows_shared), stream_ptr()), "dmp_seg_sum2")
    else:
        with _lib.timed("seg_sum[H=%d,rows=%d,ent=%d]", (H, num_nodes, nent), nbytes):
            check(lib.dmp_seg_sum(ptr(M), ldm, ptr(rowptr), ptr(ent), ptr(ew), num_nodes, H,
                                  ptr(out), ldo, int(rows_shared), stream_ptr()), "dmp_seg_sum")
    return out


def gather_rows_raw(X, idx32, edge_w=None):
    lib = _lib.load()
    _lib.require_gpu(X, idx32, edge_w)
    X, ldx = _mat(X)
    E, H = idx32.numel(), X.size(1)
    out = torch.empty((E, H), dtype=torch.float32, device=X.device)
    ew = _vec(edge_w, torch.float32)
    with _lib.timed("gather_rows[H=%d,E=%d]", (H, E), 4 * H * (E + X.size(0)) + 4 * E):
        check(lib.dmp_gather_rows(ptr(X), ldx, ptr(idx32), ptr(ew), E, H, ptr(out), H, stream_ptr()),
              "dmp_gather_rows")
    return out


def gather_select_raw(D, dst32, rev8, H, edge_w=None, s0=1.0, s1=1.0, base=None):
    lib = _lib.load()
    _lib.require_gpu(D, dst32, rev8, edge_w, base)
    D, ldd = _mat(D)
    E = dst32.numel()
    out = torch.empty((E, H), dtype=torch.float32, device=D.device)
    ew = _vec(edge_w, torch.float32)
    ldb = 0
    if base is not None:
        base, ldb = _mat(base)
    nbytes = 4 * H * (E + 2 * D.size(0)) + 5 * E + (4 * H * E if base is not None else 0)
    with _lib.timed("gather_select%s[H=%d,E=%d]", ("+base" if base is not None else "", H, E), nbytes):
        check(lib.dmp_gather_select(ptr(D), ldd, ptr(dst32), ptr(rev8), ptr(ew), ptr(base), ldb, E, H, s0, s1,
                                    ptr(out), H, stream_ptr()), "dmp_gather_select")
    return out


class _SegSum(torch.autograd.Function):

    @staticmethod
    def forward(ctx, M, index, edge_w):
        ctx.index = index
        ctx.edge_w = edge_w
        return seg_sum_raw(M, index.in_ptr, index.in_ent, index.num_nodes, edge_w)

    @staticmethod
    @once_differentiable
    def backward(ctx, dA):
        return gather_rows_raw(dA, ctx.index.dst32, ctx.edge_w), None, None


class _SegSumBySrc(torch.autograd.Function):

    @staticmethod
    def forward(ctx, M, index):
        ctx.index = index
        return seg_sum_raw(M, index.out_ptr, index.out_ent, index.num_nodes)
# ... 588 lines not shown
```

include/dmp_hip.h:

```cpp
#ifndef DMP_HIP_H
#define DMP_HIP_H

#include <stddef.h>
#include <stdint.h>

#ifdef __cplusplus
extern "C" {
#endif

#define DMP_OK 0
#define DMP_ERR_BAD_ARG (-1)
#define DMP_ERR_UNSUPPORTED (-2)
#define DMP_ERR_HIP (-3)

#define DMP_ABI_VERSION 97
int dmp_abi_version(void);
const char *dmp_last_hip_error(void);


size_t dmp_csr_workspace_words(int64_t num_nodes, int64_t num_edges);

int dmp_csr_build(const int64_t *key, const uint8_t *flag, int64_t num_edges,
                  int64_t num_nodes, int32_t *rowptr, int32_t *ent,
                  int32_t *key32, int64_t *degree, int32_t *status,
// ... 81 lines not shown
} dmp_pool_job;
#define DMP_POOL_MAX_JOBS 4
int dmp_pool_index_jobs(const dmp_pool_job *jobs, int n, void *stream);
int dmp_pool_weight_sums(const float *w, const uint8_t *flag8, const int64_t *off, int64_t B, float *out, void *stream);


int dmp_dual_subisomorphisms(const int64_t *sub, int64_t T, const int64_t *sample_ptr, const int64_t *work_ptr,
                             int64_t work_total, int64_t B, const int64_t *p_node_off, const int64_t *p_edge_off,
                             const int64_t *p_src, const int64_t *p_dst, const int64_t *p_label, int64_t PE,
                             const int64_t *g_node_off, const int64_t *g_edge_off, const int32_t *g_out_ptr,
                             const int32_t *g_out_ent, const int32_t *g_dst, const int64_t *g_label,
                             int32_t *workspace, int64_t *first_sorted, int64_t *out, int32_t *status, void *stream);
int dmp_pattern_edge_active(const int64_t *p_src, const int64_t *p_dst, const int64_t *p_edge_off,
                            const int32_t *p_edge_graph, int64_t PE, uint8_t *active, void *stream);
int dmp_subiso_edge_weights(const int64_t *sub, int64_t T, const int64_t *sample_ptr,
                            const int64_t *work_ptr, int64_t B, const int64_t *p_node_off,
                            const int64_t *p_edge_off, const int64_t *p_src, const int64_t *p_dst,
                            const int64_t *p_label, const uint8_t *active, const int64_t *g_node_off,
                            const int32_t *g_out_ptr, const int32_t *g_out_ent, const int32_t *g_dst,
                            const int64_t *g_label, int64_t *out, int64_t E, int64_t work_hint,
                            int32_t *status, void *stream);

size_t dmp_class_tiles_workspace_words(int64_t num_nodes, int num_classes);
int dmp_class_tiles(const int64_t *deg, const int32_t *in_ptr, const int32_t *in_ent, int64_t num_nodes,
                    int64_t num_edges, int num_classes, int64_t tiles_bound, int32_t *ws,
                    int32_t *slot_edge, float *tile_scale, int32_t *num_tiles, void *stream);
int dmp_class_tiles_gated(const int64_t *deg, const int32_t *in_ptr, const int32_t *in_ent, const float *gate, int32_t *row_cnt,
                          int64_t num_nodes, int64_t num_edges, int num_classes, int64_t tiles_bound, int32_t *ws,
                          int32_t *slot_edge, float *tile_scale, int32_t *num_tiles, void *stream);

int64_t dmp_csr_keep_scratch_words(int64_t num_nodes);
int dmp_csr_keep(const int32_t *in_ptr, const int32_t *in_ent, const float *gate, int64_t num_nodes, int64_t num_entries,
                 int32_t *row_cnt, int32_t *keep_ptr, int32_t *keep_ent, void *stream);

size_t dmp_scan_workspace_words(int64_t n);
int dmp_exclusive_scan_i64(const int64_t *in, int64_t n, int64_t *out,
                           int64_t *ws, void *stream);


int dmp_seg_sum(const float *M, int64_t ldm, const int32_t *rowptr,
                const int32_t *ent, const float *edge_w, int64_t num_nodes,
                int H, float *out, int64_t ldo, int rows_shared, void *stream);

int dmp_seg_sum2_tiled(const float *M, int64_t ldm, const int32_t *rowptr, const int32_t *ent,
                       const int64_t *node_off, const int64_t *edge_off, int64_t Ba, int64_t Bb, int ka, int kb,
                       int H, float s0, float s1, float *out, int64_t ldo, void *stream);
int dmp_seg_sum2(const float *M, int64_t ldm, const int32_t *rowptr,
                 const int32_t *ent, const float *edge_w, int64_t num_nodes,
                 int H, float s0, float s1, float *out, int64_t ldo,
                 int rows_shared, void *stream);
int dmp_seg_sum2_rows(const float *M, int64_t ldm, const int32_t *rowptr, const int32_t *ent, const int32_t *rowlist,
                      const int32_t *rowcount, int ptr_by_pos, int incidence, int64_t num_nodes, int H, float s0, float s1, float *out,
                      int64_t ldo, void *stream);
int dmp_incidence_keep(const int32_t *in_ptr, const int32_t *in_ent, const int32_t *out_ptr, const int32_t *out_ent,
                       const float *gate, const int32_t *list, const int32_t *count, int64_t num_nodes, int32_t *row_cnt,
                       int32_t *keep_ptr, int32_t *keep_ent, void *stream);

int dmp_gate_compact_hist_nodes(void);
int dmp_gate_compact(const float *gate, const int64_t *src, const int64_t *dst, const uint8_t *rev, const int64_t *node_off,
                     const int64_t *edge_off, int64_t B, int64_t N, int64_t E, int64_t cap, int zero_deg, int32_t *kept,
                     int64_t *out_deg, int64_t *src_c, int64_t *dst_c, uint8_t *rev_c, int64_t *eid_map, float *gate_c,
                     int64_t *num_edges_c, int64_t *edge_off_c, int32_t *status, void *stream);
int dmp_out_degrees(const int64_t *src, int64_t E, int64_t N, int64_t *deg, void *stream);

int dmp_seg_sum2_graphs_max_nodes(void);
int dmp_seg_sum2_graphs(const float *M, int64_t ldm, const int32_t *sel_a, const int32_t *sel_b,
                        const int64_t *node_off, const int64_t *edge_off, int64_t Ba, int64_t Bb, int ka, int kb,
                        int H, float s0, float s1, float *out, int64_t ldo, void *stream);
int dmp_seg_sum2_graphs_masked(const float *M, int64_t ldm, const int32_t *sel_a, const int32_t *sel_b,
                               const int64_t *node_off, const int64_t *edge_off, int64_t Ba, int64_t Bb, int ka, int kb,
                               int H, float s0, float s1, float *out, int64_t ldo, const uint32_t *rowmask, int64_t num_rows,
                               const uint32_t *nodemask, int64_t num_nodes, void *stream);

int dmp_gather_rows(const float *X, int64_t ldx, const int32_t *idx,
                    const float *edge_w, int64_t num_edges, int H, float *out,
                    int64_t ldo, void *stream);

int dmp_gather_select(const float *D, int64_t ldd, const int32_t *dst,
                      const uint8_t *flag, const float *edge_w,
                      const float *base, int64_t ldb, int64_t num_edges, int H,
                      float s0, float s1, float *out, int64_t ldo, void *stream);

int dmp_edge_combine(const float *G, int64_t ldg, const float *P, int64_t ldp,
                     const float *coef, const float *bias, const int32_t *src,
                     const int32_t *dst, const uint8_t *flag,
                     int64_t num_edges, int H, int relu, float slope, float *Y, int64_t ldy,
                     void *stream);

int dmp_edge_combine_bwd_g(const float *dY, int64_t ldy, const float *coef,
                           const int32_t *dst, int64_t num_edges, int H,
                           float *dG, int64_t ldg, void *stream);

int dmp_compgcn_agg(const float *X, int64_t ldx, const float *Z, int64_t ldz,
                    const int32_t *rowptr, const int32_t *ent,
                    const int32_t *src, const float *norm, int64_t num_nodes,
                    int H, int comp, float *out, int64_t ldo, void *stream);

int dmp_compgcn_agg_bwd(const float *D, int64_t ldd, const float *X,
                        int64_t ldx, const float *Z, int64_t ldz,
                        const int32_t *src, const int32_t *dst,
                        const uint8_t *flag, const float *norm,
                        int64_t num_edges, int H, int comp, float *dZ,
                        int64_t lddz, float *dXe, int64_t lddxe, void *stream);


int64_t dmp_colsum_partial_rows(int64_t rows, int H);

int dmp_gate_residual(const float *prev, int64_t ldp, const float *upd, int64_t ldu,
                      const float *gate, int64_t rows, int H, float *out, int64_t ldo,
                      void *stream);

int dmp_add_bias_relu(const float *a, int64_t lda, const float *b, int64_t ldb, const float *bias,
                      int64_t rows, int H, float slope, float *out, int64_t ldo, void *stream);

int dmp_scale_rows_colsum(const float *dOut, int64_t ldd, const float *gate, int64_t rows,
                          int H, float *dUpd, int64_t ldu, float *partial, void *stream);

int dmp_relu_bwd_colsum(const float *dH, int64_t ldh, const float *act, int64_t lda,
                        int64_t rows, int H, float slope, float *dPre, int64_t ldp, float *partial,
                        void *stream);

int dmp_relu_bwd_gathered_colsum(const float *table, int64_t ldt, const int32_t *rowmap, const float *gate, const float *act,
                                 int64_t lda, int64_t R, int H, float slope, float *dPre, int64_t ldp, float *partial, void *stream);

int64_t dmp_pool_relu_bwd_blocks(int64_t num_chunks, int H);
int dmp_pool_relu_bwd(const float *act, int64_t lda, const float *table, int64_t ldt, const int32_t *rowmap, const float *gate,
                      const int32_t *vptr, const int32_t *vent, int64_t num_chunks, int64_t R, int H, float slope, float *dPre,
                      int64_t ldp, float *chunk_sums, float *partial, void *stream);

int dmp_edge_combine_bwd_g_colsum(const float *dY, int64_t ldy, const float *coef,
                                  const int32_t *dst, int64_t num_edges, int H, float *dG,
                                  int64_t ldg, float *partial, void *stream);

int dmp_relu_bwd_g_colsum(const float *dH, int64_t ldh, const float *act, int64_t lda,
                          const float *coef, const int32_t *dst, int64_t num_edges, int H, float slope,
                          float *dG, int64_t ldg, float *partial, void *stream);

int dmp_colsum_partials(const float *A, int64_t lda, int64_t rows, int H, float *partial,
                        void *stream);

int dmp_smallk_embed_gate(const float *X, int64_t ldx, int K, const float *W, int64_t ldw,
                          const float *gate, int64_t rows, int H, float *out, int64_t ldo, void *stream);
int dmp_smallk_embed_live(const float *X, int64_t ldx, int K, const float *W, int64_t ldw, const float *gate, int64_t R,
                          int H, float *out, int64_t ldo, void *stream);
int dmp_smallk_embed_cols(const float *X, int64_t ldx, int K, const float *W, int64_t ldw, const float *gate,
                          int64_t rows, int H, int ncols, float *out, int64_t ldo, void *stream);
int dmp_smallk_atb_cols_masked(const float *X, int64_t ldx, int K, const float *D, int64_t ldd, int ncols, const float *D2,
                               int64_t ldd2, const float *gate, const uint32_t *rowmask, int64_t R, int H, float *partial,
                               void *stream);
int dmp_smallk_atb_cols_rows(const float *X, int64_t ldx, int K, const float *D, int64_t ldd, int ncols, const float *D2,
                             int64_t ldd2, const int32_t *list, const int32_t *count, int64_t R, int H, float *partial, void *stream);
typedef struct {
  const float *X; int64_t ldx;
  const float *D; int64_t ldd;
  const float *gate;
  const uint32_t *rowmask;
  int64_t R;
  float *partial;
} dmp_smallk_job;
int dmp_smallk_atb_jobs(const dmp_smallk_job *jobs, int num_jobs, int K, int H, void *stream);
int64_t dmp_smallk_atb_blocks(int64_t rows);
int dmp_smallk_atb(const float *X, int64_t ldx, int K, const float *D, int64_t ldd, const float *gate,
                   int64_t rows, int H, float *partial, void *stream);

int dmp_l0_pack(const float *enc_p, int64_t ldp, int64_t rows_p, const float *enc_g, int64_t ldg, const float *gate,
                int64_t rows_g, int K, int Kpad, int goff, float *out, void *stream);
typedef struct {
  const float *enc_p; int64_t ldp; int64_t rows_p;
  const float *enc_g; int64_t ldg; const float *gate; int64_t rows_g;
  int K, Kpad, goff;
  float *out;
} dmp_l0_pack_job;
int dmp_l0_pack_jobs(const dmp_l0_pack_job *jobs, int num_jobs, void *stream);
int dmp_l0_edge_fwd_masked(const float *enc, int64_t lde, int K, const float *M, int64_t ldm, const float *P, int64_t ldp,
                           const float *bias, const float *coef_e, const int32_t *sel_a, const int32_t *sel_b,
                           const uint32_t *rowmask, int64_t R, int H, float slope, float *out, int64_t ldo, void *stream);
int64_t dmp_l0_node_pack_rows(void);
int dmp_l0_node_fwd(const float *venc, int64_t ldv, int VK, const float *S0, int64_t lds, int K0, int Kp, const float *W, int64_t ldw,
                    const float *bias, float slope, const uint32_t *rowmask, const int32_t *list, const int32_t *count, int64_t list_bound,
                    int64_t q_begin, int64_t n0, int64_t n1, int H, float *h1, int64_t ldh, float *P, int64_t ldp, void *stream);
int dmp_l0_node_fwd_mfma_max_codes(void);
// ... 189 lines not shown
int dmp_edge_select_nodes(const int32_t *src, const int32_t *dst, const uint8_t *flag, const uint32_t *nodemask,
                          int64_t num_edges, int32_t *selA, int32_t *selB, int32_t *dstM, void *stream);

int dmp_edge_fwd_fused(const float *Z, int64_t ldz, const float *W, int64_t ldw,
                       const float *P, int64_t ldp, int64_t num_nodes, const float *bias,
                       const int32_t *selA, const int32_t *selB, const float *coefE,
                       int64_t num_edges, int H, float slope, float *H1, int64_t ldh, void *stream);


int64_t dmp_mfma_partial_rows_h(int64_t num_edges, int H);

int dmp_row_mask_bits(const float *gate, int64_t E, uint32_t *mask, void *stream);
int dmp_row_mask_rows(const float *X, int64_t ldx, int K, int64_t R, uint32_t *mask, void *stream);

int dmp_out_fwd_fused_rows(const float *Hin, int64_t ldh, const float *W2, int64_t ldw, const float *bias,
                           const float *gate, const uint32_t *rowmask, int dead_rows, const float *R, int64_t ldr, int64_t E, int H,
                           int w_in_out, float *out, int64_t ldo, void *stream);
int dmp_bwd_h1_fused_rows(const float *dO, int64_t ldo, const float *W2, int64_t ldw, const float *H1, int64_t ldh,
                          const float *coefE, const float *gate, const uint32_t *rowmask, int skip_dead_stores, int64_t E, int H,
                          float slope, float *dG, int64_t ldg, float *partial, float *partial_rows, void *stream);

int64_t dmp_typed_partial_rows(int64_t tiles_bound, int H);
typedef struct {
  const float *Hin; int64_t ldh;
  const float *W2; int64_t ldw; int w_in_out;
  const float *bias;
  const float *R; int64_t ldr;
  const float *R2; int64_t ldr2;
  int act; float slope;
  float *out; int64_t ldo;
} dmp_typed_job;
int dmp_out_fwd_typed(const dmp_typed_job *jobs, int num_jobs, const int32_t *slot_edge, const float *tile_scale,
                      const int32_t *num_tiles, int64_t tiles_bound, int64_t E, int H, void *stream);
int dmp_bwd_h1_typed(const float *dO, int64_t ldo, const float *W2, int64_t ldw, const float *H1, int64_t ldh,
                     const int32_t *slot_edge, const float *tile_scale, const int32_t *num_tiles, int64_t tiles_bound, int64_t E,
                     int H, float slope, float *dG, int64_t ldg, float *partial, float *partial_rows, void *stream);
int dmp_out_fwd_typed_codes(const dmp_typed_job *job, const float *codes, int64_t ldc, int kcodes, const float *Wc, int64_t ldwc,
                            int64_t code_row0, int64_t r_rows, const int32_t *slot_edge, const float *tile_scale, const int32_t *num_tiles, int64_t tiles_bound, int64_t E,
                            int H, void *stream);

typedef struct {
  const float *Z; int64_t ldz;
  const float *D; int64_t ldd;
  float *partial_T, *partial_B; int64_t partial_stride; int ldp;
} dmp_atb2_job;
int64_t dmp_atb2_blocks(int64_t tiles_bound, int num_jobs);
int dmp_atb2_jobs(const dmp_atb2_job *jobs, int num_jobs, const int32_t *slot_row, const float *tile_scale, const int32_t *num_tiles,
                  int64_t tiles_bound, int64_t rows, int H, void *stream);

int dmp_bwd_z_w(const float *dPre, int64_t ldp, const float *Z, int64_t ldz, const float *W, int64_t ldw, const float *D, int64_t ldd,
                int64_t num_nodes, const float *base, int64_t ldb, const int32_t *dst, const uint8_t *flag, float s0, float s1,
                const int32_t *slot_edge, const float *tile_scale, const int32_t *num_tiles, int64_t tiles_bound, int64_t E, int H,
                const int32_t *base_map, int64_t base_rows, float *dZ, int64_t ldo, float *partial_w, void *stream);
int64_t dmp_bwd_h1_w_blocks(int64_t tiles_bound);
int dmp_bwd_h1_w(const float *dO, int64_t ldo, const float *W2, int64_t ldw, const float *H1, int64_t ldh,
                 const int32_t *slot_edge, const int32_t *num_tiles, int64_t tiles_bound, int64_t E, int H, float slope,
                 float *dG, int64_t ldg, float *partial, float *partial_rows, float *partial_w, void *stream);
int dmp_bwd_h1_w_max_codes(void);
int dmp_bwd_h1_w_codes(const float *dO, int64_t ldo, const float *W2, int64_t ldw, const float *H1, int64_t ldh,
                       const int32_t *slot_edge, const int32_t *num_tiles, int64_t tiles_bound, int64_t E, int H, float slope,
                       float *dG, int64_t ldg, float *partial, float *partial_rows, float *partial_w,
                       const float *enc, int64_t lde, int K, const float *coef_e, int64_t r0, int64_t r1, int residual,
                       float *partial_x, void *stream);

typedef struct {
  const float *W; int64_t ld; int transposed;
} dmp_chain_panel;
int64_t dmp_node_chain_blocks(int64_t tiles_bound);
int64_t dmp_node_chain_panel_words(void);
int dmp_node_chain_pack(const dmp_chain_panel *panels, int num_panels, uint32_t *out, void *stream);
int dmp_node_chain_fwd(const float *x, int64_t ldx, const float *S, int64_t lds, const uint32_t *panels, const float *bn, const float *b2,
                       int residual, float slope, const int32_t *slot, const int32_t *num_tiles, int64_t tiles_bound, int64_t rows, int H,
                       float *H1n, int64_t ldh, float *P, int64_t ldp, float *xn, int64_t ldxn, void *stream);
int dmp_node_chain_bwd(const float *dxn, int64_t ldd, const float *H1n, int64_t ldh, const float *dP, int64_t ldp, const uint32_t *panels,
                       int residual, float slope, const int32_t *slot, const int32_t *num_tiles, int64_t tiles_bound, int64_t rows, int H,
                       float *dPn, int64_t ldn, float *dS, int64_t lds, float *dx, int64_t ldx, float *partial, float *partial_rows,
                       void *stream);

int dmp_edge_mlp_fwd(const float *Z, int64_t ldz, const float *W, int64_t ldw, const float *P, int64_t ldp, int64_t num_nodes,
                     const float *bias1, const int32_t *selA, const int32_t *selB, const float *W2, int64_t ldw2, int w2_in_out,
                     const float *bias2, const float *R, int64_t ldr, const int32_t *slot_edge, const float *tile_scale,
                     const int32_t *num_tiles, int64_t tiles_bound, int64_t num_edges, int H, float slope, float *H1, int64_t ldh,
                     float *out, int64_t ldo, void *stream);

int dmp_l0_edge_mlp_max_codes(void);
int dmp_l0_edge_mlp_fwd(const float *enc, int64_t lde, int K, const float *M, int64_t ldm, int tables, int64_t row_split, const float *P,
                        int64_t ldp, int64_t num_nodes, const float *bias1, const float *coefE, const int32_t *selA, const int32_t *selB,
                        float slope, const float *W2, int64_t ldw2, int w2_in_out, const float *bias2, const float *Wc, int64_t ldwc,
                        int64_t code_row0, const float *R, int64_t ldr, int64_t r_rows, const int32_t *slot_edge, const int32_t *num_tiles,
                        int64_t tiles_bound, int64_t num_edges, int H, float *H1, int64_t ldh, float *out, int64_t ldo, void *stream);

int dmp_bwd_z_fused(const float *dPre, int64_t ldp, const float *W, int64_t ldw,
                    const float *D, int64_t ldd, int64_t num_nodes, const float *base, int64_t ldb,
                    const float *coefE, const int32_t *dst, const uint8_t *flag, float s0,
                    float s1, int64_t num_edges, int H, float *dZ, int64_t ldz, void *stream);

int dmp_edge_fwd_typed(const float *Z, int64_t ldz, const float *W, int64_t ldw, const float *P,
                       int64_t ldp, int64_t num_nodes, const float *bias, const int32_t *selA,
                       const int32_t *selB, const int32_t *slot_edge, const float *tile_scale,
                       const int32_t *num_tiles, int64_t tiles_bound, int64_t num_edges, int H,
                       float slope, float *H1, int64_t ldh, void *stream);
int dmp_mask_slots(const int32_t *slot, int64_t n, const float *gate, int64_t E, int32_t *out, void *stream);
int dmp_bwd_z_typed_arow(const float *dPre, int64_t ldp, const float *W, int64_t ldw, const float *D, int64_t ldd,
                         int64_t num_nodes, const float *base, int64_t ldb, const int32_t *dst, const uint8_t *flag,
                         float s0, float s1, const int32_t *slot_edge, const int32_t *slot_arow, const float *tile_scale,
                         const int32_t *num_tiles, int64_t tiles_bound, int64_t E, int H, int w_transposed,
// ... 147 lines not shown
```

Baseline: 534,800.

## Store dPre as activation sign bits and rebuild it from U in consumers

The pool ReLU backward no longer writes the full dense dPre matrix. It writes a 16-byte sign mask per edge row, and the consumers (the segment-sum endpoint kernel and the dZ/W backward GEMM) rebuild dPre on the fly from the compact table U, the row map and the leaky slope. This removes a large f32 write and its later reads in exchange for extra gathers of U rows and sign words in each consumer. It adds a gated path with many preconditions and new kernel variants, and the GEMM load pipeline gains extra scalar loads and DPP shuffles.

```diff
diff --git a/dualmessagepassing_amd/_abi.py b/dualmessagepassing_amd/_abi.py
--- a/dualmessagepassing_amd/_abi.py
+++ b/dualmessagepassing_amd/_abi.py
@@ -335,6 +335,12 @@
     "dmp_atb2_jobs": (c_int, [_p(dmp_atb2_job), c_int, c_ptr, c_ptr, c_ptr, c_i64, c_i64, c_int, c_ptr]),
     "dmp_bwd_z_w": (c_int, [c_ptr, c_i64, c_ptr, c_i64, c_ptr, c_i64, c_ptr, c_i64, c_i64, c_ptr, c_i64, c_ptr, c_ptr, c_f32, c_f32,
                             c_ptr, c_ptr, c_ptr, c_i64, c_i64, c_int, c_ptr, c_i64, c_ptr, c_i64, c_ptr, c_ptr]),
+    "dmp_bwd_z_w_signs": (c_int, [c_ptr, c_ptr, c_ptr, c_i64, c_i64, c_f32, c_ptr, c_i64, c_ptr, c_i64, c_ptr, c_i64, c_i64, c_ptr, c_i64,
+                                  c_ptr, c_ptr, c_f32, c_f32, c_ptr, c_ptr, c_ptr, c_i64, c_i64, c_int, c_ptr, c_i64, c_ptr, c_i64, c_ptr, c_ptr]),
+    "dmp_pool_relu_bwd_signs": (c_int, [c_ptr, c_i64, c_ptr, c_i64, c_ptr, c_ptr, c_ptr, c_ptr, c_i64, c_i64, c_int, c_f32, c_ptr, c_ptr,
+                                        c_ptr, c_ptr]),
+    "dmp_seg_sum2_rows_signs": (c_int, [c_ptr, c_ptr, c_i64, c_ptr, c_f32, c_ptr, c_ptr, c_ptr, c_ptr, c_int, c_i64, c_int, c_f32, c_f32,
+                                        c_ptr, c_i64, c_ptr]),
     "dmp_out_fwd_typed_codes": (c_int, [_p(dmp_typed_job), c_ptr, c_i64, c_int, c_ptr, c_i64, c_i64, c_i64, c_ptr, c_ptr, c_ptr, c_i64, c_i64, c_int, c_ptr]),
     "dmp_bwd_h1_w_blocks": (c_i64, [c_i64]),
     "dmp_bwd_h1_w": (c_int, [c_ptr, c_i64, c_ptr, c_i64, c_ptr, c_i64, c_ptr, c_ptr, c_i64, c_i64, c_int, c_f32, c_ptr, c_i64,
diff --git a/dualmessagepassing_amd/csrc/dmp_agg.hip b/dualmessagepassing_amd/csrc/dmp_agg.hip
--- a/dualmessagepassing_amd/csrc/dmp_agg.hip
+++ b/dualmessagepassing_amd/csrc/dmp_agg.hip
@@ -108,6 +108,57 @@
       }
     }
   }
+}
+
+template <int BLOCK = kBlock>
+__global__ __launch_bounds__(BLOCK) void seg_sum_signs_k(
+    const uint32_t *__restrict__ signs, const float *__restrict__ U, int64_t ldu, const int32_t *__restrict__ rowmap, float slope,
+    const int32_t *__restrict__ rowptr, const int32_t *__restrict__ ent, int N, float s0, float s1, float *__restrict__ out,
+    int64_t ldo, const int32_t *__restrict__ rowlist, const int32_t *__restrict__ rowcount, int ptr_by_pos) {
+  constexpr int G = 32, H = 128, RPB = BLOCK / G, UNR = 8;
+  const int nwg = (*rowcount + RPB - 1) / RPB;
+  if ((int)blockIdx.x >= nwg) return;
+  int row = xcd_remap(blockIdx.x, nwg) * RPB + threadIdx.x / G;
+  const int lane = threadIdx.x % G;
+  if (row >= N || row >= *rowcount) return;
+  int prow = row;
+  row = rowlist[row];
+  if (!ptr_by_pos) prow = row;
+  const int beg = rowptr[prow], end = rowptr[prow + 1];
+  const int c = lane * 4;
+  float4 a0 = zero4(), a1 = zero4();
+  for (int base = beg; base < end; base += G) {
+    const int cnt = min(G, end - base);
+    int my = 0, mym = -1;
+    if (lane < cnt) {
+      my = ent[base + lane];
+      mym = rowmap[my >> 1];
+    }
+    for (int j = 0; j < cnt; j += UNR) {
+      float4 v[UNR];
+      uint32_t w[UNR];
+      int e[UNR];
+#pragma unroll
+      for (int k = 0; k < UNR; ++k) {
+        e[k] = __shfl(my, min(j + k, G - 1), G);
+        const int m = __shfl(mym, min(j + k, G - 1), G);
+        if (j + k < cnt) {
+          w[k] = signs[(int64_t)(e[k] >> 1) * kSignWords + (lane >> 3)];
+          v[k] = m >= 0 ? ld4(U + (int64_t)m * ldu + c) : zero4();
+        }
+      }
+#pragma unroll
+      for (int k = 0; k < UNR; ++k) {
+        if (j + k < cnt) {
+          const float4 d = dpre_from_signs(sign_nibble_of(w[k], lane), v[k], slope);
+          if (e[k] & 1) add4(a1, d); else add4(a0, d);
+        }
+      }
+    }
+  }
+  float *o = out + (int64_t)row * ldo + c;
+  st4(o, mul4(a0, s0));
+  st4(o + H, mul4(a1, s1));
 }
 
 constexpr int kTileRows = 512, kTileCols = 32, kTilePad = 36, kTileThreads = 512;
@@ -647,6 +698,18 @@
                       ptr_by_pos ? 1 : 0);
 }
 
+int dmp_seg_sum2_rows_signs(const uint32_t *signs, const float *U, int64_t ldu, const int32_t *rowmap, float slope, const int32_t *rowptr,
+                            const int32_t *ent, const int32_t *rowlist, const int32_t *rowcount, int ptr_by_pos, int64_t num_nodes, int H,
+                            float s0, float s1, float *out, int64_t ldo, void *stream) {
+  if (num_nodes < 0 || H <= 0 || ldu < H || ldo < 2 * H || !(slope >= 0.f && slope <= 1.f)) return DMP_ERR_BAD_ARG;
+  if (num_nodes == 0) return DMP_OK;
+  if (!signs || !U || !rowmap || !rowptr || !ent || !rowlist || !rowcount || !out) return DMP_ERR_BAD_ARG;
+  if (H != 128 || num_nodes >= kMaxRows || !vec_ok(H, {ldu, ldo}, {U, out})) return DMP_ERR_UNSUPPORTED;
+  seg_sum_signs_k<<<blocks_for(num_nodes, kBlock / 32), kBlock, 0, (hipStream_t)stream>>>(
+      signs, U, ldu, rowmap, slope, rowptr, ent, (int)num_nodes, s0, s1, out, ldo, rowlist, rowcount, ptr_by_pos ? 1 : 0);
+  return check_launch();
+}
+
 int dmp_seg_sum2_tiled(const float *M, int64_t ldm, const int32_t *rowptr, const int32_t *ent, const int64_t *node_off,
                        const int64_t *edge_off, int64_t Ba, int64_t Bb, int ka, int kb, int H, float s0, float s1,
                        float *out, int64_t ldo, void *stream) {
diff --git a/dualmessagepassing_amd/csrc/dmp_common.h b/dualmessagepassing_amd/csrc/dmp_common.h
--- a/dualmessagepassing_amd/csrc/dmp_common.h
+++ b/dualmessagepassing_amd/csrc/dmp_common.h
@@ -49,4 +49,13 @@
 __device__ __forceinline__ float act_fwd(float x, float a) { return fmaxf(x, a * x); }
 __device__ __forceinline__ float act_bwd(float y, float d, float a) { return y > 0.f ? d : a * d; }
 
+constexpr int kSignWords = 4;
+__device__ __forceinline__ uint32_t sign_nibble(const float4 &y) {
+  return (y.x > 0.f ? 1u : 0u) | (y.y > 0.f ? 2u : 0u) | (y.z > 0.f ? 4u : 0u) | (y.w > 0.f ? 8u : 0u);
 }
+__device__ __forceinline__ uint32_t sign_nibble_of(uint32_t word, int l) { return (word >> (4 * (l & 7))) & 15u; }
+__device__ __forceinline__ float4 dpre_from_signs(uint32_t nib, const float4 &u, float a) {
+  return make_float4((nib & 1u) ? u.x : a * u.x, (nib & 2u) ? u.y : a * u.y, (nib & 4u) ? u.z : a * u.z, (nib & 8u) ? u.w : a * u.w);
+}
+
+}
diff --git a/dualmessagepassing_amd/csrc/dmp_fused.hip b/dualmessagepassing_amd/csrc/dmp_fused.hip
--- a/dualmessagepassing_amd/csrc/dmp_fused.hip
+++ b/dualmessagepassing_amd/csrc/dmp_fused.hip
@@ -541,6 +541,7 @@
   const float *h1; int64_t ldh; const float *table; int64_t ldt; const int32_t *rowmap; const float *gate;
   const int32_t *vptr, *vent; int64_t V; int H; float slope;
   float *dpre; int64_t ldp; float *qc; float *partial;
+  uint32_t *signs;
 };
 
 template <int G>
@@ -603,6 +604,70 @@
   }
 }
 
+__global__ __launch_bounds__(kBlock) void pool_relu_signs_k(PoolBwdArgs p) {
+  constexpr int G = 32, GPB = kBlock / G, UNR = 8;
+  __shared__ float4 red[kBlock];
+  const int grp = threadIdx.x / G, lane = threadIdx.x % G;
+  const int c = lane * 4;
+  float4 cs = zero4();
+  for (int64_t ch = (int64_t)blockIdx.x * GPB + grp; ch < p.V; ch += (int64_t)gridDim.x * GPB) {
+    const int beg = p.vptr[ch], end = p.vptr[ch + 1];
+    float4 q0 = zero4(), q1 = zero4();
+    for (int base = beg; base < end; base += G) {
+      const int cnt = min(G, end - base);
+      int ent = 0, mi = -1;
+      float gt = 0.f;
+      if (lane < cnt) {
+        ent = p.vent[base + lane];
+        const int r = ent >> 1;
+        mi = p.rowmap[r];
+        gt = p.gate ? p.gate[r] : 1.f;
+      }
+      for (int j = 0; j < cnt; j += UNR) {
+        float4 hv[UNR], uv[UNR];
+        int en[UNR];
+        float sc[UNR];
+#pragma unroll
+        for (int k = 0; k < UNR; ++k) {
+          en[k] = __shfl(ent, min(j + k, G - 1), G);
+          const int tr = __shfl(mi, min(j + k, G - 1), G);
+          sc[k] = __shfl(gt, min(j + k, G - 1), G);
+          if (j + k < cnt) {
+            const bool live = sc[k] != 0.f;
+            hv[k] = live ? ld4(p.h1 + (int64_t)(en[k] >> 1) * p.ldh + c) : zero4();
+            uv[k] = (live && tr >= 0) ? ld4(p.table + (int64_t)tr * p.ldt + c) : zero4();
+          }
+        }
+#pragma unroll
+        for (int k = 0; k < UNR; ++k)
+          if (j + k < cnt) {
+            const float4 u = mul4(uv[k], sc[k]);
+            const float4 t = make_float4(act_bwd(hv[k].x, u.x, p.slope), act_bwd(hv[k].y, u.y, p.slope),
+                                         act_bwd(hv[k].z, u.z, p.slope), act_bwd(hv[k].w, u.w, p.slope));
+            uint32_t w = sign_nibble(hv[k]) << (4 * (lane & 7));
+            w |= (uint32_t)__shfl_xor((int)w, 1, G);
+            w |= (uint32_t)__shfl_xor((int)w, 2, G);
+            w |= (uint32_t)__shfl_xor((int)w, 4, G);
+            if ((lane & 7) == 0) p.signs[(int64_t)(en[k] >> 1) * kSignWords + (lane >> 3)] = w;
+            add4(cs, t);
+            const float4 gh = mul4(hv[k], sc[k]);
+            if (en[k] & 1) add4(q1, gh); else add4(q0, gh);
+          }
+      }
+    }
+    st4(p.qc + ch * 2 * p.H + c, q0);
+    st4(p.qc + ch * 2 * p.H + p.H + c, q1);
+  }
+  red[threadIdx.x] = cs;
+  __syncthreads();
+  if (grp == 0) {
+    float4 t = red[lane];
+#pragma unroll
+    for (int g = 1; g < GPB; ++g) add4(t, red[g * G + lane]);
+    st4(p.partial + (int64_t)blockIdx.x * p.H + c, t);
+  }
+}
+
 template <int OP>
 int launch_rowop(const RowArgs &p, hipStream_t st) {
   const int g = group_lanes(p.H);
@@ -703,12 +768,28 @@
   DMP_ROW_CHECK(h1 && table && rowmap && vptr && vent && dPre && chunk_sums && ldh >= H && ldt >= H && ldp >= H);
   if (!vec_shape_ok(H, ldh, ldt, ldp) || H > 256 || !ok16(h1) || !ok16(table) || !ok16(dPre) || !ok16(chunk_sums) || !ok16(partial))
     return DMP_ERR_UNSUPPORTED;
-  PoolBwdArgs p{h1, ldh, table, ldt, rowmap, gate, vptr, vent, num_chunks, H, slope, dPre, ldp, chunk_sums, partial};
+  PoolBwdArgs p{h1, ldh, table, ldt, rowmap, gate, vptr, vent, num_chunks, H, slope, dPre, ldp, chunk_sums, partial, nullptr};
   hipStream_t st = (hipStream_t)stream;
   const int g = group_lanes(H);
   if (g == 16) pool_relu_bwd_k<16><<<(unsigned)nb, kBlock, 0, st>>>(p);
   else if (g == 32) pool_relu_bwd_k<32><<<(unsigned)nb, kBlock, 0, st>>>(p);
   else pool_relu_bwd_k<64><<<(unsigned)nb, kBlock, 0, st>>>(p);
+  return check_launch();
+}
+
+int dmp_pool_relu_bwd_signs(const float *h1, int64_t ldh, const float *table, int64_t ldt, const int32_t *rowmap, const float *gate,
+                            const int32_t *vptr, const int32_t *vent, int64_t num_chunks, int64_t R, int H, float slope, uint32_t *signs,
+                            float *chunk_sums, float *partial, void *stream) {
+  DMP_ROW_CHECK(R >= 0 && num_chunks >= 0 && H > 0 && partial);
+  if (!slope_ok(slope) || H != 128) return DMP_ERR_UNSUPPORTED;
+  const int64_t nb = dmp_pool_relu_bwd_blocks(num_chunks, H);
+  if (R == 0 || num_chunks == 0)
+    return hipMemsetAsync(partial, 0, sizeof(float) * (size_t)H * (size_t)nb, (hipStream_t)stream) == hipSuccess ? DMP_OK : DMP_ERR_HIP;
+  DMP_ROW_CHECK(h1 && table && rowmap && vptr && vent && signs && chunk_sums && ldh >= H && ldt >= H);
+  if (!vec_shape_ok(H, ldh, ldt, 0) || !ok16(h1) || !ok16(table) || !ok16(signs) || !ok16(chunk_sums) || !ok16(partial))
+    return DMP_ERR_UNSUPPORTED;
+  PoolBwdArgs p{h1, ldh, table, ldt, rowmap, gate, vptr, vent, num_chunks, H, slope, nullptr, 0, chunk_sums, partial, signs};
+  pool_relu_signs_k<<<(unsigned)nb, kBlock, 0, (hipStream_t)stream>>>(p);
   return check_launch();
 }
 
diff --git a/dualmessagepassing_amd/csrc/dmp_h1w.hip b/dualmessagepassing_amd/csrc/dmp_h1w.hip
--- a/dualmessagepassing_amd/csrc/dmp_h1w.hip
+++ b/dualmessagepassing_amd/csrc/dmp_h1w.hip
@@ -667,8 +667,10 @@
   const int32_t *rmap; int64_t rowsR;
   float s0, s1;
   float *partialW; int64_t pstride;
+  const uint32_t *signs; const int32_t *smap; const float *U; int64_t ldu; int64_t rowsU; float slope;
 };
 
+template <bool SIGNS>
 __global__ __launch_bounds__(kThreadsW, 1) void dzw_k(const DzwArgs p) {
   extern __shared__ __attribute__((aligned(256))) unsigned char lds[];
   float *const scr_all = reinterpret_cast<float *>(lds + kImgB);
@@ -687,9 +689,11 @@
   const int hi = lo + chunk < ntiles ? lo + chunk : ntiles;
   const int mine = hi > lo ? hi - lo : 0;
   const rsrc_t rs_slot = make_rsrc(p.slot_edge, (uint32_t)ntiles * (kSub * 4u));
-  const srsrc_t rs_X = cols ? make_srsrc(p.Z, p.ldz, p.E) : make_srsrc(p.dPre, p.ldp, p.E);
+  const srsrc_t rs_X = cols ? make_srsrc(p.Z, p.ldz, p.E) : (SIGNS ? make_srsrc(p.U, p.ldu, p.rowsU) : make_srsrc(p.dPre, p.ldp, p.E));
   const uint32_t op_off = cols ? (uint32_t)kOpB : 0u;
   const uint32_t rows4 = (uint32_t)(p.E * 4);
+  const rsrc_t rs_smap = make_rsrc(p.smap, SIGNS ? rows4 : 0u);
+  const rsrc_t rs_sign = make_rsrc(p.signs, SIGNS ? rows4 * (uint32_t)kSignWords : 0u);
   const rsrc_t rs_dst = make_rsrc(p.dst, rows4);
   const rsrc_t rs_flag = make_rsrc(p.flag, p.flag ? (uint32_t)p.E : 0u);
   const rsrc_t rs_rmap = make_rsrc(p.rmap, p.rmap ? rows4 : 0u);
@@ -709,12 +713,37 @@
   auto load_ids = [&](int k) {
     const bool ok = k < mine;
     const uint32_t so = (uint32_t)(lo + k) * (kSub * 4u);
-#pragma unroll
-    for (int m = 0; m < kSubLoads; ++m)
-      id_rows[m] = ok ? (int)__builtin_amdgcn_raw_buffer_load_b32(rs_slot, (srow + 8 * m) * 4, (int)so, 0) : -1;
+    if (!SIGNS || cols) {
+#pragma unroll
+      for (int m = 0; m < kSubLoads; ++m)
+        id_rows[m] = ok ? (int)__builtin_amdgcn_raw_buffer_load_b32(rs_slot, (srow + 8 * m) * 4, (int)so, 0) : -1;
+    }
     if (!cols && u < kSub) id_own = ok ? (int)__builtin_amdgcn_raw_buffer_load_b32(rs_slot, u * 4, (int)so, 0) : -1;
   };
   auto load_row = [&](int m) { pre[m] = sbuf_load4(rs_X, id_rows[m], (uint32_t)scol * 16u); };
+  int id_sel = -1, sg_map = -1;
+  uint32_t sg_word = 0, sg_nibs = 0;
+  auto sg_load_id = [&](int k) {
+    id_sel = k < mine ? (int)__builtin_amdgcn_raw_buffer_load_b32(rs_slot, (srow + 8 * (scol & 3)) * 4, (int)((uint32_t)(lo + k) * (kSub * 4u)), 0) : -1;
+  };
+  auto sg_load_scalars = [&]() {
+    const bool ok = id_sel >= 0;
+    const int m = (int)__builtin_amdgcn_raw_buffer_load_b32(rs_smap, ok ? (int)((uint32_t)id_sel * 4u) : (int)kOOB, 0, 0);
+    sg_word = __builtin_amdgcn_raw_buffer_load_b32(rs_sign, ok ? (int)((uint32_t)id_sel * 16u + (uint32_t)(scol >> 3) * 4u) : (int)kOOB, 0, 0);
+    sg_map = ok ? m : -1;
+  };
+  auto sg_load_row = [&](auto mc) {
+    constexpr int m = decltype(mc)::value;
+    const int rm = __builtin_amdgcn_mov_dpp(sg_map, 0x55 * m, 0xF, 0xF, false);
+    const uint32_t w = (uint32_t)__builtin_amdgcn_mov_dpp((int)sg_word, 0x55 * m, 0xF, 0xF, false);
+    pre[m] = sbuf_load4(rs_X, rm, (uint32_t)scol * 16u);
+    const uint32_t nb = sign_nibble_of(w, scol) << (4 * m);
+    sg_nibs = m == 0 ? nb : (sg_nibs | nb);
+  };
+  auto sg_load_rows = [&]() {
+    sg_load_row(std::integral_constant<int, 0>{}); sg_load_row(std::integral_constant<int, 1>{});
+    sg_load_row(std::integral_constant<int, 2>{}); sg_load_row(std::integral_constant<int, 3>{});
+  };
   auto load_row_scalars = [&]() {
     if (!cols && u < kSub) {
       const uint32_t eo = id_own >= 0 ? (uint32_t)id_own * 4u : kOOB;
@@ -726,8 +755,10 @@
   };
   auto stage_row = [&](int buf, int m) {
     uint2 ph, pm, pl;
-    split_pair(pre[m].x, pre[m].y, ph.x, pm.x, pl.x);
-    split_pair(pre[m].z, pre[m].w, ph.y, pm.y, pl.y);
+    float4 v = pre[m];
+    if (SIGNS && !cols) v = dpre_from_signs((sg_nibs >> (4 * m)) & 15u, v, p.slope);
+    split_pair(v.x, v.y, ph.x, pm.x, pl.x);
+    split_pair(v.z, v.w, ph.y, pm.y, pl.y);
     const uint32_t r = (uint32_t)(srow + 8 * m);
     const uint32_t off = op_off + (uint32_t)buf * kBufB + 256u * r + 16u * ((uint32_t)(scol >> 1) ^ swz(r)) + 8u * (uint32_t)(scol & 1);
     *reinterpret_cast<uint2 *>(lds + off) = ph;
@@ -754,8 +785,17 @@
   };
 
   load_ids(0);
-#pragma unroll
-  for (int m = 0; m < kSubLoads; ++m) load_row(m);
+  if (SIGNS && !cols) {
+    sg_load_id(0);
+    sg_load_scalars();
+    sg_load_id(1);
+    sg_load_rows();
+    sg_load_scalars();
+    sg_load_id(2);
+  } else {
+#pragma unroll
+    for (int m = 0; m < kSubLoads; ++m) load_row(m);
+  }
   load_row_scalars();
   load_ids(1);
 
@@ -916,9 +956,19 @@
       if (i < 4) {}
       else if (i < 8) stage_row(buf ^ 1, i - 4);
       else if (i == 8) stage_scalars(nxt3);
-      else if (i < 13) load_row(i - 9);
+      else if (i < 13) {
+        if constexpr (SIGNS) {
+          if (i == 9) sg_load_row(std::integral_constant<int, 0>{});
+          else if (i == 10) sg_load_row(std::integral_constant<int, 1>{});
+          else if (i == 11) sg_load_row(std::integral_constant<int, 2>{});
+          else sg_load_row(std::integral_constant<int, 3>{});
+        } else {
+          load_row(i - 9);
+        }
+      }
       else if (i == 13) load_row_scalars();
       else if (i == 14) load_ids(k + 3);
+      else if (i == 15) { if constexpr (SIGNS) { sg_load_scalars(); sg_load_id(k + 4); } }
     };
 #pragma unroll
     for (int g = 0; g < kGroups; ++g) {
@@ -963,8 +1013,14 @@
 #pragma unroll
   for (int m = 0; m < kSubLoads; ++m) stage_row(0, m);
   stage_scalars(0);
-#pragma unroll
-  for (int m = 0; m < kSubLoads; ++m) load_row(m);
+  if constexpr (SIGNS) {
+    sg_load_rows();
+    sg_load_scalars();
+    sg_load_id(3);
+  } else {
+#pragma unroll
+    for (int m = 0; m < kSubLoads; ++m) load_row(m);
+  }
   load_row_scalars();
   load_ids(2);
   lds_barrier();
@@ -989,9 +1045,10 @@
 }
 
 constexpr int kDzwLdsBytes = kImgB + kScrB + 4 * 3 * kSub * 4;
+template <bool SIGNS>
 inline bool dzw_lds_ready() {
   static bool done[kMaxDevices] = {};
-  return opt_in_lds(reinterpret_cast<const void *>(&dzw_k), kDzwLdsBytes, done);
+  return opt_in_lds(reinterpret_cast<const void *>(&dzw_k<SIGNS>), kDzwLdsBytes, done);
 }
 
 inline unsigned h1w_blocks(int64_t tiles_bound) { return one_per_cu_blocks(tiles_bound); }
@@ -1107,13 +1164,45 @@
       num_nodes >= ((int64_t)1 << 31) || tiles_bound * kSub * 4 >= ((int64_t)1 << 32) - 8192 || (int64_t)H * ldw * 4 >= ((int64_t)1 << 32) - 8192 ||
       !fits4g(E, ldp) || !fits4g(E, ldz) || !fits4g(E, ldo) || (base && !fits4g(base_map ? base_rows : E, ldb)) || !fits4g(num_nodes, ldd))
     return DMP_ERR_UNSUPPORTED;
-  if (!dzw_lds_ready()) return DMP_ERR_HIP;
+  if (!dzw_lds_ready<false>()) return DMP_ERR_HIP;
   DzwArgs a{};
   a.dPre = dPre; a.ldp = ldp; a.Z = Z; a.ldz = ldz; a.W = W; a.ldw = ldw; a.dZ = dZ; a.ldo = ldo; a.E = E; a.slot_edge = slot_edge;
   a.tile_scale = tile_scale; a.num_tiles = num_tiles; a.dst = dst; a.flag = flag; a.D = D; a.ldd = ldd; a.num_nodes = num_nodes;
   a.base = base; a.ldb = base ? ldb : H; a.rmap = base_map; a.rowsR = base_rows; a.s0 = s0; a.s1 = s1;
   a.partialW = partial_w; a.pstride = (int64_t)H * 2 * H;
-  dzw_k<<<h1w_blocks(tiles_bound), kThreadsW, kDzwLdsBytes, st>>>(a);
+  dzw_k<false><<<h1w_blocks(tiles_bound), kThreadsW, kDzwLdsBytes, st>>>(a);
+  return check_launch();
+}
+
+int dmp_bwd_z_w_signs(const uint32_t *signs, const int32_t *sign_map, const float *U, int64_t ldu, int64_t rows_u, float slope,
+                      const float *Z, int64_t ldz, const float *W, int64_t ldw, const float *D, int64_t ldd, int64_t num_nodes,
+                      const float *base, int64_t ldb, const int32_t *dst, const uint8_t *flag, float s0, float s1,
+                      const int32_t *slot_edge, const float *tile_scale, const int32_t *num_tiles, int64_t tiles_bound, int64_t E, int H,
+                      const int32_t *base_map, int64_t base_rows, float *dZ, int64_t ldo, float *partial_w, void *stream) {
+  if (H != 128 || g_exact_fp32) return DMP_ERR_UNSUPPORTED;
+  if (E < 0 || num_nodes < 0 || tiles_bound < 0 || rows_u < 0 || !partial_w || !aligned16(partial_w)) return DMP_ERR_BAD_ARG;
+  if (!(slope >= 0.f && slope <= 1.f)) return DMP_ERR_UNSUPPORTED;
+  hipStream_t st = (hipStream_t)stream;
+  if (E == 0) return hipMemsetAsync(partial_w, 0, sizeof(float) * H * 2 * H * (size_t)h1w_blocks(tiles_bound), st) == hipSuccess ? DMP_OK : DMP_ERR_HIP;
+  if (!signs || !sign_map || !U || !Z || !W || !D || !dst || !slot_edge || !tile_scale || !num_tiles || !dZ || ldu < H || ldz < H ||
+      ldw < 2 * H || ldd < 2 * H || ldo < H || (base && ldb < H))
+    return DMP_ERR_BAD_ARG;
+  if (base_map && (!base || base_rows < 0)) return DMP_ERR_BAD_ARG;
+  if (ldu % 4 || ldz % 4 || ldo % 4 || ldd % 4 || (base && ldb % 4) || !aligned16(U) || !aligned16(Z) || !aligned16(dZ) || !aligned16(D) ||
+      (base && !aligned16(base)) || (reinterpret_cast<uintptr_t>(signs) & 3u))
+    return DMP_ERR_UNSUPPORTED;
+  if (!stride_ok(ldu) || !stride_ok(ldz) || !stride_ok(ldo) || !stride_ok(ldd) || (base && !stride_ok(ldb)) || E >= ((int64_t)1 << 27) ||
+      num_nodes >= ((int64_t)1 << 31) || tiles_bound * kSub * 4 >= ((int64_t)1 << 32) - 8192 || (int64_t)H * ldw * 4 >= ((int64_t)1 << 32) - 8192 ||
+      !fits4g(rows_u, ldu) || !fits4g(E, ldz) || !fits4g(E, ldo) || (base && !fits4g(base_map ? base_rows : E, ldb)) || !fits4g(num_nodes, ldd))
+    return DMP_ERR_UNSUPPORTED;
+  if (!dzw_lds_ready<true>()) return DMP_ERR_HIP;
+  DzwArgs a{};
+  a.Z = Z; a.ldz = ldz; a.W = W; a.ldw = ldw; a.dZ = dZ; a.ldo = ldo; a.E = E; a.slot_edge = slot_edge;
+  a.tile_scale = tile_scale; a.num_tiles = num_tiles; a.dst = dst; a.flag = flag; a.D = D; a.ldd = ldd; a.num_nodes = num_nodes;
+  a.base = base; a.ldb = base ? ldb : H; a.rmap = base_map; a.rowsR = base_rows; a.s0 = s0; a.s1 = s1;
+  a.partialW = partial_w; a.pstride = (int64_t)H * 2 * H;
+  a.signs = signs; a.smap = sign_map; a.U = U; a.ldu = ldu; a.rowsU = rows_u; a.slope = slope;
+  dzw_k<true><<<h1w_blocks(tiles_bound), kThreadsW, kDzwLdsBytes, st>>>(a);
   return check_launch();
 }
 
diff --git a/dualmessagepassing_amd/fused.py b/dualmessagepassing_amd/fused.py
--- a/dualmessagepassing_amd/fused.py
+++ b/dualmessagepassing_amd/fused.py
@@ -119,7 +119,7 @@
     return out, reduce_partials(part)
 
 
-def pool_relu_bwd(table, rowmap, gate, act, pool, slope=0.0, skip_dead=False, chunk_sums=False):
+def pool_relu_bwd(table, rowmap, gate, act, pool, slope=0.0, skip_dead=False, chunk_sums=False, signs=False):
     lib = _lib.load()
     R, H = act.shape
     V = pool.num_chunks
@@ -127,11 +127,18 @@
     part = torch.empty((nb, H), dtype=torch.float32, device=act.device)
     kc = keep_pool_csr(pool, gate) if skip_dead else None
     vptr, vent = (pool.vptr, pool.vent) if kc is None else kc
-    out = dead_rows_buffer((R, H), act.device) if kc is not None else torch.empty((R, H), dtype=torch.float32, device=act.device)
     qc = torch.empty((V, 2 * H), dtype=torch.float32, device=act.device)
-    with _lib.timed("pool_relu_bwd[H=%d,R=%d]", (H, R), 8 * H * R + 12 * R + 8 * H * V):
-        check(lib.dmp_pool_relu_bwd(ptr(act), act.stride(0), ptr(table), table.stride(0), ptr(rowmap), ptr(gate), ptr(vptr),
-                                    ptr(vent), V, R, H, slope, ptr(out), H, ptr(qc), ptr(part), stream_ptr()), "dmp_pool_relu_bwd")
+    if signs:
+        out = dead_rows_buffer((R, 4), act.device).view(torch.int32) if kc is not None else torch.empty((R, 4), dtype=torch.int32, device=act.device)
+        nbytes = signs_record_bytes((4 * H + 16 + 12) * R + 8 * H * V, kc is not None)
+        with _lib.timed("pool_relu_bwd[H=%d,signs=%d]", (H, R), nbytes):
+            check(lib.dmp_pool_relu_bwd_signs(ptr(act), act.stride(0), ptr(table), table.stride(0), ptr(rowmap), ptr(gate), ptr(vptr),
+                                              ptr(vent), V, R, H, slope, ptr(out), ptr(qc), ptr(part), stream_ptr()), "dmp_pool_relu_bwd_signs")
+    else:
+        out = dead_rows_buffer((R, H), act.device) if kc is not None else torch.empty((R, H), dtype=torch.float32, device=act.device)
+        with _lib.timed("pool_relu_bwd[H=%d,R=%d]", (H, R), 8 * H * R + 12 * R + 8 * H * V):
+            check(lib.dmp_pool_relu_bwd(ptr(act), act.stride(0), ptr(table), table.stride(0), ptr(rowmap), ptr(gate), ptr(vptr),
+                                        ptr(vent), V, R, H, slope, ptr(out), H, ptr(qc), ptr(part), stream_ptr()), "dmp_pool_relu_bwd")
     if chunk_sums:
         return out, reduce_partials(part), qc
     Q = ops.seg_sum_raw(qc, pool.gptr, pool.gent, pool.num_graphs, None, False, rows_shared=False)
@@ -462,13 +469,24 @@
     return out
 
 
-def bwd_z_w(d_pre, z, Wes, d_s, base, coef, index, WesT=None, base_map=None, gate=None, dead_rows=None, dst=None):
-    lib = _lib.load()
-    E, H = d_pre.size(0), Wes.size(0)
+def signs_record_bytes(shape_bytes, gated):
+    return 0 if gated else shape_bytes
+
+
+class DPreSigns:
+    __slots__ = ("mask", "U", "rowmap", "slope")
+
+    def __init__(self, mask, U, rowmap, slope):
+        self.mask, self.U, self.rowmap, self.slope = mask, U, rowmap, float(slope)
+
+
+def bwd_z_w_tiles(E, H, z, d_s_cols, base, coef, index, gate, dead_rows, d_pre=None):
+    lib = _lib.load()
     lim = (1 << 32) - 65536
     if ((dead_rows is None) != (gate is None) or H != 128 or lib.dmp_dev_get_exact_fp32() or z is None or z.size(0) != E or E * H * 4 >= lim
-            or E * d_pre.stride(0) * 4 >= lim or E * z.stride(0) * 4 >= lim or d_pre.data_ptr() % 16 or z.data_ptr() % 16
-            or d_pre.stride(0) % 4 or z.stride(0) % 4 or index.num_nodes * d_s.size(1) * 4 >= lim):
+            or E * z.stride(0) * 4 >= lim or z.data_ptr() % 16 or z.stride(0) % 4 or index.num_nodes * d_s_cols * 4 >= lim):
+        return None
+    if d_pre is not None and (E * d_pre.stride(0) * 4 >= lim or d_pre.data_ptr() % 16 or d_pre.stride(0) % 4):
         return None
     if gate is None:
         if getattr(index, "_coef_deg", None) is None or index._coef_deg[0] is not coef or index.num_edges == 0:
@@ -480,19 +498,36 @@
         return None
     if base is not None and (base.stride(0) % 4 or base.data_ptr() % 16 or base.size(0) * base.stride(0) * 4 >= lim):
         return None
+    return lt
+
+
+def bwd_z_w(d_pre, z, Wes, d_s, base, coef, index, WesT=None, base_map=None, gate=None, dead_rows=None, dst=None):
+    lib = _lib.load()
+    sg = d_pre if isinstance(d_pre, DPreSigns) else None
+    E, H = (z.size(0) if sg is not None else d_pre.size(0)), Wes.size(0)
+    lt = bwd_z_w_tiles(E, H, z, d_s.size(1), base, coef, index, gate, dead_rows, None if sg is not None else d_pre)
+    if lt is None:
+        if sg is not None:
+            raise _lib.DmpError("bwd_z_w: dPre was handed over as sign bits, but the two-role kernel does not apply")
+        return None
     slot_edge, tile_scale, num_tiles, bound = lt
-    out = (torch.zeros((E, H), dtype=torch.float32, device=d_pre.device) if dead_rows == "zero" else
-           dead_rows_buffer((E, H), d_pre.device) if dead_rows == "leave" else torch.empty((E, H), dtype=torch.float32, device=d_pre.device))
+    out = (torch.zeros((E, H), dtype=torch.float32, device=z.device) if dead_rows == "zero" else
+           dead_rows_buffer((E, H), z.device) if dead_rows == "leave" else torch.empty((E, H), dtype=torch.float32, device=z.device))
     if WesT is None:
         WesT = torch.cat([Wes[:, :H].t(), Wes[:, H:].t()], dim=1)
     d_s = d_s.contiguous()
     G = int(lib.dmp_bwd_h1_w_blocks(bound))
-    part = torch.empty((G, H * 2 * H), dtype=torch.float32, device=d_pre.device)
-    with _lib.timed("bwd_z_w[H=%d,E=%d]", (H, E), 4 * H * E * (4 if base is not None else 3) + 5 * E):
-        check(lib.dmp_bwd_z_w(ptr(d_pre), d_pre.stride(0), ptr(z), z.stride(0), ptr(WesT), WesT.size(1), ptr(d_s), d_s.size(1), index.num_nodes,
-                              ptr(base), base.stride(0) if base is not None else H, ptr(index.dst32 if dst is None else dst), ptr(index.rev8), -1.0, 1.0,
-                              ptr(slot_edge), ptr(tile_scale), ptr(num_tiles), bound, E, H, ptr(base_map),
-                              base.size(0) if base_map is not None else 0, ptr(out), H, ptr(part), stream_ptr()), "dmp_bwd_z_w")
+    part = torch.empty((G, H * 2 * H), dtype=torch.float32, device=z.device)
+    tail = (ptr(z), z.stride(0), ptr(WesT), WesT.size(1), ptr(d_s), d_s.size(1), index.num_nodes,
+            ptr(base), base.stride(0) if base is not None else H, ptr(index.dst32 if dst is None else dst), ptr(index.rev8), -1.0, 1.0,
+            ptr(slot_edge), ptr(tile_scale), ptr(num_tiles), bound, E, H, ptr(base_map),
+            base.size(0) if base_map is not None else 0, ptr(out), H, ptr(part), stream_ptr())
+    if sg is not None:
+        with _lib.timed("bwd_z_w_signs[H=%d,E=%d]", (H, E), signs_record_bytes(4 * H * E * (3 if base is not None else 2) + 25 * E, gate is not None)):
+            check(lib.dmp_bwd_z_w_signs(ptr(sg.mask), ptr(sg.rowmap), ptr(sg.U), sg.U.stride(0), sg.U.size(0), sg.slope, *tail), "dmp_bwd_z_w_signs")
+    else:
+        with _lib.timed("bwd_z_w[H=%d,E=%d]", (H, E), 4 * H * E * (4 if base is not None else 3) + 5 * E):
+            check(lib.dmp_bwd_z_w(ptr(d_pre), d_pre.stride(0), *tail), "dmp_bwd_z_w")
     return out, reduce_partials(part).view(H, 2 * H)
 
 
@@ -1883,13 +1918,35 @@
     return XX, dict(enc=c.l0.enc, K=K0, coef_e=c.index.edge_select(c.coef)[2], rows=rows, residual=c.residual, out=XX[t * K0:(t + 1) * K0])
 
 
-def _edge_out_bwd_lazy(c, H1e, lazy, gcnt):
+USE_DPRE_SIGNS = True
+
+
+def dpre_signs_ok(c, z, lazy, typed, want_dz):
+    ix, H, e_gate = c.index, c.H, c.e_gate
+    if not (USE_DPRE_SIGNS and lazy is not None and c.poolalg and H == 128 and c.l0 is None and typed and want_dz):
+        return False
+    if e_gate is not None and binary_gate_mask(e_gate) is None:
+        return False
+    if not (e_gate is None or dead_edge_rows(ix, H, e_gate, c.coef)):
+        return False
+    if not kept_incidence_sums(ix, H, e_gate, c.nd is not None):
+        return False
+    T = lazy[0]
+    base = T if c.residual else None
+    dead_dz = (("leave" if (c.inner & 2) else "zero") if dead_edge_rows(ix, H, e_gate) else None)
+    return bwd_z_w_tiles(z.size(0), H, z, 2 * H, base, c.coef, ix, e_gate, dead_dz) is not None
+
+
+def _edge_out_bwd_lazy(c, H1e, lazy, gcnt, signs=False):
     H, e_gate = c.H, c.e_gate
     T, emap, ep = lazy
     if c.poolalg:
         T = T if _aligned(T) else T.clone(memory_format=torch.contiguous_format)
         skip = c.l0 is None and c.nd is not None and USE_PLAIN_ATB and dead_edge_rows(c.index, H, e_gate, c.coef)
-        dG, dbe, qc = pool_relu_bwd(rows_gemm(T, c.eW2, False), emap, e_gate, H1e, ep, c.slope, skip_dead=skip, chunk_sums=True)
+        U = rows_gemm(T, c.eW2, False)
+        dG, dbe, qc = pool_relu_bwd(U, emap, e_gate, H1e, ep, c.slope, skip_dead=skip, chunk_sums=True, signs=signs)
+        if signs:
+            dG = DPreSigns(dG, U, emap, c.slope)
         if gcnt is None:
             gcnt = pool_weight_sums(ep, e_gate)
         dW2e, db2e = pool_wgrad(qc, ep, T, gcnt)
@@ -1934,9 +1991,9 @@
     return dG, dbe, dW2e, db2e, l0_XX
 
 
-def _edge_out_bwd(c, tables, H1e, dzn, lazy, gcnt, typed):
+def _edge_out_bwd(c, tables, H1e, dzn, lazy, gcnt, typed, signs=False):
     if lazy is not None:
-        return _edge_out_bwd_lazy(c, H1e, lazy, gcnt) + (None,)
+        return _edge_out_bwd_lazy(c, H1e, lazy, gcnt, signs) + (None,)
     if typed:
         return _edge_out_bwd_typed(c, tables, H1e, dzn)
     dOe, db2e = scale_rows_colsum(dzn, c.e_gate)
@@ -1952,6 +2009,9 @@
     sums_masked = typed and USE_MASKED_SUMS and has_row_mask(e_gate)
     if kept_incidence_sums(ix, H, e_gate, nd is not None):
         kp, ke = nd.kept_incidence(ix, e_gate)
+        if isinstance(dG, DPreSigns):
+            ops.seg_sum_signs(dG.mask, dG.U, dG.rowmap, dG.slope, kp, ke, N, 1.0, -1.0, dXP[:, H:], nd.rows)
+            return dXP
         ops.seg_sum_raw(dG[:, :H], kp, ke, N, None, True, 1.0, -1.0, out=dXP[:, H:], rows=nd.rows, ptr_by_pos=True, tag="seg_sum2_kept_inc",
                         incidence=True)
     else:
@@ -1976,6 +2036,8 @@
     ix, H, e_gate = c.index, c.H, c.e_gate
     if typed and want_dz and H == 128 and (e_gate is None or dead_edge_rows(ix, H, e_gate, c.coef)):
         return None
+    if isinstance(dG, DPreSigns):
+        raise _lib.DmpError("fused layer backward: dPre as sign bits without the launch that reads them")
     return atb_typed(z, dG, c.coef, ix, gate=e_gate) if typed else atb(z, dG)
 
 
@@ -2233,7 +2295,8 @@
         dxn, dzn, lazy = _grad_seeds(c, x, z, H1e, dxn, dzn, dvs, des, typed)
         dz = dW0 = dWV0 = None
         with deferred_reductions():
-            dG, dbe, dW2e, db2e, l0_XX = _edge_out_bwd(c, tables, H1e, dzn, lazy, ctx.gcnt, typed)
+            signs = dpre_signs_ok(c, z, lazy, typed, want_dz)
+            dG, dbe, dW2e, db2e, l0_XX = _edge_out_bwd(c, tables, H1e, dzn, lazy, ctx.gcnt, typed, signs)
             dXP = _endpoint_sums(c, dG, typed, x.device)
             if c.l0 is not None:
                 XX = _l0_edge_code_products(c, tables, dG, dzn, l0_XX)
diff --git a/dualmessagepassing_amd/ops.py b/dualmessagepassing_amd/ops.py
--- a/dualmessagepassing_amd/ops.py
+++ b/dualmessagepassing_amd/ops.py
@@ -134,6 +134,22 @@
         with _lib.timed("seg_sum[H=%d,rows=%d,ent=%d]", (H, num_nodes, nent), nbytes):
             check(lib.dmp_seg_sum(ptr(M), ldm, ptr(rowptr), ptr(ent), ptr(ew), num_nodes, H,
                                   ptr(out), ldo, int(rows_shared), stream_ptr()), "dmp_seg_sum")
+    return out
+
+
+def seg_sum_signs(mask, U, rowmap, slope, rowptr, ent, num_nodes, s0, s1, out, rows, ptr_by_pos=True, gated=True):
+    lib = _lib.load()
+    _lib.require_gpu(mask, U, rowmap, rowptr, ent)
+    H = U.size(1)
+    if out.shape != (num_nodes, 2 * H) or out.dtype != torch.float32 or (num_nodes > 1 and out.stride(1) != 1):
+        raise _lib.DmpError("seg_sum_signs: bad out tensor")
+    ldo = out.stride(0) if num_nodes > 1 else 2 * H
+    nent = ent.numel()
+    nbytes = 0 if gated else 24 * nent + 8 * H * num_nodes + 12 * num_nodes
+    with _lib.timed("seg_sum2_signs[H=%d,rows=%d,ent=%d]", (H, num_nodes, nent), nbytes):
+        check(lib.dmp_seg_sum2_rows_signs(ptr(mask), ptr(U), U.stride(0), ptr(rowmap), float(slope), ptr(rowptr), ptr(ent), ptr(rows[0]),
+                                          ptr(rows[1]), int(bool(ptr_by_pos)), num_nodes, H, s0, s1, ptr(out), ldo, stream_ptr()),
+              "dmp_seg_sum2_rows_signs")
     return out
 
 
diff --git a/include/dmp_hip.h b/include/dmp_hip.h
--- a/include/dmp_hip.h
+++ b/include/dmp_hip.h
@@ -157,6 +157,9 @@
 int dmp_seg_sum2_rows(const float *M, int64_t ldm, const int32_t *rowptr, const int32_t *ent, const int32_t *rowlist,
                       const int32_t *rowcount, int ptr_by_pos, int incidence, int64_t num_nodes, int H, float s0, float s1, float *out,
                       int64_t ldo, void *stream);
+int dmp_seg_sum2_rows_signs(const uint32_t *signs, const float *U, int64_t ldu, const int32_t *rowmap, float slope, const int32_t *rowptr,
+                            const int32_t *ent, const int32_t *rowlist, const int32_t *rowcount, int ptr_by_pos, int64_t num_nodes, int H,
+                            float s0, float s1, float *out, int64_t ldo, void *stream);
 int dmp_incidence_keep(const int32_t *in_ptr, const int32_t *in_ent, const int32_t *out_ptr, const int32_t *out_ent,
                        const float *gate, const int32_t *list, const int32_t *count, int64_t num_nodes, int32_t *row_cnt,
                        int32_t *keep_ptr, int32_t *keep_ent, void *stream);
@@ -232,6 +235,9 @@
 int dmp_pool_relu_bwd(const float *act, int64_t lda, const float *table, int64_t ldt, const int32_t *rowmap, const float *gate,
                       const int32_t *vptr, const int32_t *vent, int64_t num_chunks, int64_t R, int H, float slope, float *dPre,
                       int64_t ldp, float *chunk_sums, float *partial, void *stream);
+int dmp_pool_relu_bwd_signs(const float *act, int64_t lda, const float *table, int64_t ldt, const int32_t *rowmap, const float *gate,
+                            const int32_t *vptr, const int32_t *vent, int64_t num_chunks, int64_t R, int H, float slope, uint32_t *signs,
+                            float *chunk_sums, float *partial, void *stream);
 
 int dmp_edge_combine_bwd_g_colsum(const float *dY, int64_t ldy, const float *coef,
                                   const int32_t *dst, int64_t num_edges, int H, float *dG,
@@ -527,6 +533,11 @@
                 int64_t num_nodes, const float *base, int64_t ldb, const int32_t *dst, const uint8_t *flag, float s0, float s1,
                 const int32_t *slot_edge, const float *tile_scale, const int32_t *num_tiles, int64_t tiles_bound, int64_t E, int H,
                 const int32_t *base_map, int64_t base_rows, float *dZ, int64_t ldo, float *partial_w, void *stream);
+int dmp_bwd_z_w_signs(const uint32_t *signs, const int32_t *sign_map, const float *U, int64_t ldu, int64_t rows_u, float slope,
+                      const float *Z, int64_t ldz, const float *W, int64_t ldw, const float *D, int64_t ldd, int64_t num_nodes,
+                      const float *base, int64_t ldb, const int32_t *dst, const uint8_t *flag, float s0, float s1,
+                      const int32_t *slot_edge, const float *tile_scale, const int32_t *num_tiles, int64_t tiles_bound, int64_t E, int H,
+                      const int32_t *base_map, int64_t base_rows, float *dZ, int64_t ldo, float *partial_w, void *stream);
 int64_t dmp_bwd_h1_w_blocks(int64_t tiles_bound);
 int dmp_bwd_h1_w(const float *dO, int64_t ldo, const float *W2, int64_t ldw, const float *H1, int64_t ldh,
                  const int32_t *slot_edge, const int32_t *num_tiles, int64_t tiles_bound, int64_t E, int H, float slope,
```

Measured after the change: 539,600 (median of 6 runs). About the same (+0.9%).
